# chongchen1999/llm-inference-engine

Measured on AMD Instinct MI355X. Metric: decode_tokens_per_s, higher is better.
Workload: dtype f16; 1 GPU; Llama-2-7B 32-layer fp16 decode, batch 1, ctx 2048 (BASELINE configs[2]); random-init weights, synthetic ids, KV pre-filled; global_batch=1, seq_len=2048, parallelism=replicas x1 (no collective), graph=True, layers=32

## Files before the change

### include/llmie.h

```cpp
#ifndef LLMIE_H
#define LLMIE_H

#include <stddef.h>
#include <stdint.h>

#ifdef __cplusplus
extern "C" {
#endif

#define LLMIE_ABI_VERSION 3

typedef enum { LLMIE_F32 = 0, LLMIE_F16 = 1 } llmie_dtype;

typedef enum {
    LLMIE_OK = 0,
    LLMIE_ERR_INVALID_ARG = -1,
    LLMIE_ERR_UNSUPPORTED = -2,
    LLMIE_ERR_LAUNCH = -3,
    LLMIE_ERR_WORKSPACE = -4
} llmie_status;

typedef void *llmie_stream;

typedef enum {
// ... 159 lines not shown
    int32_t *out_top_ids;
    float   *out_top_logprobs;
} llmie_sampling_ext;
int llmie_sample_logits_ext(const void *logits, int batch, int vocab, const llmie_sampling_params *params_dev, int32_t *history,
                            int history_stride, int32_t *history_len, int history_append, int32_t *seq_len, uint8_t *finished,
                            int32_t *out_id, float *out_logprob, int step, const int32_t *step_dev, int end_id, void *workspace,
                            size_t workspace_bytes, llmie_dtype dtype, llmie_stream stream, const llmie_sampling_ext *ext);

size_t llmie_score_tokens_workspace_bytes(int rows, int hidden_size, int vocab);
int llmie_score_tokens(const void *hidden, const void *norm_gamma, float rms_eps, const void *lm_head, const void *lm_bias,
                       const int32_t *targets, float *out_logprob, float *out_lse, int32_t *out_argmax,
                       float *out_argmax_logprob, int rows, int hidden_size, int vocab, void *workspace,
                       size_t workspace_bytes, llmie_dtype dtype, llmie_stream stream);


int llmie_linear_w8a16(const void *x, const int8_t *wq, const void *scale, void *y,
                       int M, int K, int N, const void *bias, const void *residual,
                       void *workspace, size_t workspace_bytes, llmie_stream stream);
int llmie_linear_w4a16(const void *x, const uint8_t *wq, const void *scale, void *y,
                       int M, int K, int N, int group, const void *bias, const void *residual,
                       void *workspace, size_t workspace_bytes, llmie_stream stream);
int llmie_linear_fp8(const void *x, const uint8_t *w_fp8, const float *w_scale, void *y,
                     int M, int K, int N, const void *bias, const void *residual,
                     void *workspace, size_t workspace_bytes, llmie_stream stream);
size_t llmie_linear_fp8_workspace_bytes(int M, int K, int N);
int llmie_linear_fp8_swiglu(const void *x, const uint8_t *w_fp8, const float *w_scale, void *y, int M, int K,
                            int two_inter, void *workspace, size_t workspace_bytes, llmie_stream stream);
int llmie_quantize_w8(const void *w, int8_t *wq, void *scale, int N, int K, llmie_stream stream);
int llmie_quantize_w4(const void *w, uint8_t *wq, void *scale, int N, int K, int group,
                      llmie_stream stream);
int llmie_quantize_fp8(const void *w, uint8_t *wq, float *scale, int N, int K, llmie_stream stream);

int llmie_quantize_mxfp4(const void *w, uint8_t *wq, uint8_t *scale, int N, int K, llmie_stream stream);
int llmie_dequantize_mxfp4(const uint8_t *wq, const uint8_t *scale, void *w16, int N, int K, llmie_stream stream);
int llmie_linear_mxfp4(const void *x, const uint8_t *wq, const uint8_t *scale, void *y, int M, int K, int N, const void *bias,
                       const void *residual, void *workspace, size_t workspace_bytes, llmie_stream stream);

size_t llmie_packed_weight_bytes(llmie_weight_format fmt, int N, int K, int swiglu_pairs);
size_t llmie_packed_scale_bytes(llmie_weight_format fmt, int N, int K, int swiglu_pairs);
int llmie_pack_weight(llmie_weight_format fmt, const void *w, const void *scale, void *packed, void *packed_scale,
                      int N, int K, int swiglu_pairs, llmie_stream stream);
size_t llmie_linear_packed_workspace_bytes(llmie_weight_format fmt, int M, int K, int N);
enum { LLMIE_X32_X = 1, LLMIE_X32_Y = 2, LLMIE_X32_RES = 4 };
size_t llmie_x32_bytes(int C);
int llmie_x32_convert(const void *src, void *dst, int M, int C, int to_x32, llmie_stream stream);
int llmie_linear_packed(llmie_weight_format fmt, const void *x, const void *packed, const void *scale, void *y,
                        int M, int K, int N, int swiglu, int x32_flags, const void *residual, const void *gamma,
                        const void *pre_bias, float eps, void *workspace, size_t workspace_bytes,
                        llmie_stream stream);


typedef enum { LLMIE_KV_NATIVE = 0, LLMIE_KV_FP8 = 1 } llmie_kv_format;

typedef struct {
    const void *data;
    const void *scale;
    const void *bias;
} llmie_matrix;

typedef struct {
    const void *attn_norm_gamma;
    llmie_matrix qkv;
    llmie_matrix o;
    const void *ffn_norm_gamma;
    llmie_matrix gate_up;
    llmie_matrix down;
} llmie_layer_weights;

typedef struct {
    int head_num, kv_head_num, head_size, inter_size, num_layers, vocab_size;
    int max_seq_len, max_batch;
    int rotary_dim;
    float rotary_base, rms_eps;
    llmie_dtype dtype;
    llmie_weight_format wfmt;
    int int4_group;
    llmie_kv_format kv_fmt;
    float k_scale, v_scale;
    int flags;
} llmie_decoder_config;

#define LLMIE_DEC_NO_PACKED_COPY 1
#define LLMIE_DEC_PACKED_ONLY 2
size_t llmie_decoder_resident_weight_bytes(const llmie_decoder_config *cfg);

#define LLMIE_PLAN_PAGED 1u
#define LLMIE_PLAN_RAGGED 2u
#define LLMIE_PLAN_HIDDEN_MISALIGNED 4u
#define LLMIE_PLAN_WEIGHTS_MISALIGNED 8u
#define LLMIE_PLAN_GAMMAS_MISALIGNED 16u
#define LLMIE_PLAN_O_BIAS 32u
#define LLMIE_PLAN_SCALES_MISALIGNED 64u
#define LLMIE_SW_NO_FUSED_DECODE 1u
#define LLMIE_SW_NO_FUSED_BATCH 2u
#define LLMIE_SW_NO_PACKED_BATCH 4u
#define LLMIE_SW_CHAIN 8u
#define LLMIE_SW_NO_FUSED_SHORT_PREFILL 16u
#define LLMIE_SW_NO_QKV_ROPE_FUSION 32u
const char *llmie_decoder_plan_name(const llmie_decoder_config *cfg, int prefill, int rows, unsigned call_flags, unsigned switch_mask);

#define LLMIE_PLAN_QKV_BIAS_MISALIGNED 128u
#define LLMIE_PLAN_GATE_UP_SCALES_MISALIGNED 256u
#define LLMIE_PLAN_NO_FFN_GAMMA 512u
const char *llmie_decoder_prefill_layer_plan(const llmie_decoder_config *cfg, int tokens, int batch, int max_q_len, unsigned call_flags,
                                             unsigned switch_mask, int *status);

typedef struct llmie_decoder llmie_decoder;

size_t llmie_decoder_workspace_bytes(const llmie_decoder_config *cfg);
llmie_decoder *llmie_decoder_create(const llmie_decoder_config *cfg,
                                    const llmie_layer_weights *layers,
                                    void *workspace, size_t workspace_bytes);
void llmie_decoder_destroy(llmie_decoder *dec);
int llmie_decoder_repack(llmie_decoder *dec, const llmie_layer_weights *layers, llmie_stream stream);

int llmie_decoder_forward(llmie_decoder *dec, const void *hidden_in, void *hidden_out,
                          void *k_cache, void *v_cache, int batch, int step,
                          const int32_t *step_dev, llmie_stream stream);

#define LLMIE_KV_PAGE_TOKENS 128
int llmie_decoder_forward_paged(llmie_decoder *dec, const void *hidden_in, void *hidden_out, void *k_pool, void *v_pool,
                                const int32_t *block_table, int max_pages, int num_pages, int batch, int step,
                                const int32_t *step_dev, llmie_stream stream);
int llmie_decoder_forward_ragged(llmie_decoder *dec, const void *hidden_in, void *hidden_out, void *k_cache, void *v_cache,
                                 int batch, const int32_t *ctx_len_dev, llmie_stream stream);
int llmie_decoder_forward_paged_ragged(llmie_decoder *dec, const void *hidden_in, void *hidden_out, void *k_pool, void *v_pool,
                                       const int32_t *block_table, int max_pages, int num_pages, int batch,
                                       const int32_t *ctx_len_dev, llmie_stream stream);
int llmie_decoder_prefill_paged(llmie_decoder *dec, const void *hidden_in, void *hidden_out, void *k_pool, void *v_pool,
                                const int32_t *block_table, int max_pages, int num_pages, const int32_t *input_lengths,
                                const int32_t *history_lengths, int batch, int num_tokens, int max_q_len, void *workspace,
                                size_t workspace_bytes, llmie_stream stream);
int llmie_kv_pages_copy(void *dense, void *pool, const int32_t *block_table, const int32_t *ctx_len, int to_pages,
                        int layers, int batch, int kv_head_num, int max_seq_len, int head_size, int max_pages,
                        int num_pages, int elem_bytes, llmie_stream stream);

#define LLMIE_BEAM_MAX_WIDTH 16
size_t llmie_beam_step_workspace_bytes(int groups, int width, int vocab);
int llmie_beam_step(const void *logits , int groups, int width, int vocab,
                    float *cum_logprob , int32_t *gen_len ,
                    uint8_t *finished , int32_t *out_parent ,
                    int32_t *out_token , int end_id, float length_penalty, void *workspace,
                    size_t workspace_bytes, llmie_dtype dtype, llmie_stream stream);

size_t llmie_kv_pages_fork_workspace_bytes(int rows, int layers, int kv_head_num, int head_size, int elem_bytes, int max_pages);
int llmie_kv_pages_fork(void *k_pool, void *v_pool, int32_t *block_table ,
                        const int32_t *own_table , const int32_t *parent ,
                        int32_t *cached_len , int rows, int layers, int kv_head_num, int head_size,
                        int max_pages, int num_pages, int elem_bytes, void *workspace, size_t workspace_bytes,
                        llmie_stream stream);

#define LLMIE_SPEC_MAX_DRAFT 15
size_t llmie_spec_verify_workspace_bytes(int batch, int k, int vocab);
int llmie_spec_verify(const void *logits , int batch, int k, int vocab,
                      const int32_t *draft_ids , const int32_t *draft_len ,
                      const llmie_sampling_params *params_dev , int32_t *history, int history_stride,
                      int32_t *history_len, int history_append, int32_t *seq_len, uint8_t *finished,
                      int32_t *out_tokens , int32_t *out_count , float *out_logprob ,
                      int32_t *last_token , int32_t *cached_len ,
                      int32_t *step_rows , int step, const int32_t *step_dev, int end_id,
                      void *workspace, size_t workspace_bytes, llmie_dtype dtype, llmie_stream stream,
                      const llmie_sampling_ext *ext );

int llmie_ngram_draft(const int32_t *tokens , int stride, const int32_t *len ,
                      const uint8_t *finished , int batch, int k, int max_n, int min_n, int pad_id,
                      int32_t *out_ids , int32_t *out_draft_ids ,
                      int32_t *out_draft_len , llmie_stream stream);

#define LLMIE_LORA_MAX_SLOTS 1024
#define LLMIE_LORA_MAX_KSPLIT 8
#define LLMIE_LORA_QKV 0
#define LLMIE_LORA_O 1
#define LLMIE_LORA_GATE_UP 2
#define LLMIE_LORA_DOWN 3
typedef struct {
    const void *a[4];
    const void *b[4];
} llmie_lora_layer;
typedef struct {
    int rank;
    float scale;
    int layers;
    const llmie_lora_layer *layer;
} llmie_lora_adapter;
size_t llmie_lora_table_bytes(int slots, int layers);
int llmie_lora_slot_load(void *table_dev, int slots, int layers, int slot, const llmie_lora_adapter *host_desc, llmie_stream stream);
size_t llmie_lora_workspace_bytes(int max_rows, int slots, int max_rank_total);
int llmie_lora_plan(const int32_t *slot_dev, const int32_t *lengths_dev , int batch, int rows, const void *table_dev,
                    int slots, void *workspace, size_t workspace_bytes, llmie_stream stream);
int llmie_lora_apply(const void *x , void *y , int rows, int K, int N, int blocks,
                     const int *block_widths , const void *table_dev, int slots, int layers, int layer, int module,
                     void *workspace, size_t workspace_bytes, llmie_dtype dtype, llmie_stream stream);

#define LLMIE_PLAN_LORA 1024u
size_t llmie_decoder_lora_workspace_bytes(const llmie_decoder_config *cfg, int max_tokens, int slots);
int llmie_decoder_lora_attach(llmie_decoder *dec, const void *table_dev, int slots, const int32_t *seq_slot_dev, void *workspace,
                              size_t workspace_bytes);
int llmie_decoder_lora_detach(llmie_decoder *dec);

size_t llmie_decoder_prefill_workspace_bytes(const llmie_decoder_config *cfg, int max_tokens, int max_batch);
int llmie_decoder_prefill(llmie_decoder *dec, const void *hidden_in, void *hidden_out, void *k_cache, void *v_cache,
                          const int32_t *input_lengths, const int32_t *history_lengths, int batch, int num_tokens,
                          int max_q_len, void *workspace, size_t workspace_bytes, llmie_stream stream);

int llmie_lm_head_sample(llmie_decoder *dec, void *hidden ,
                         const void *final_norm_gamma, const llmie_matrix *lm_head,
                         llmie_weight_format lm_fmt, void *logits,
                         int32_t *tmp_ids, void *tmp_vals, int32_t *topk_ids, void *topk_vals,
                         int K, int blocks_per_row, int32_t *seq_len, uint8_t *finished,
                         int32_t *out_ids, int batch, int step, const int32_t *step_dev,
                         int end_id, llmie_stream stream);

int llmie_lm_head_sample_next(llmie_decoder *dec, void *hidden, const void *final_norm_gamma, const llmie_matrix *lm_head,
                              llmie_weight_format lm_fmt, void *logits, int32_t *tmp_ids, void *tmp_vals, int32_t *topk_ids,
                              void *topk_vals, int K, int blocks_per_row, int32_t *seq_len, uint8_t *finished, int32_t *out_ids,
                              int batch, int step, int32_t *step_dev, int end_id, const void *embed_table, void *next_hidden,
                              int advance_step, llmie_stream stream);

int llmie_lm_head_sample_params(llmie_decoder *dec, void *hidden, const void *final_norm_gamma, const llmie_matrix *lm_head,
                                llmie_weight_format lm_fmt, void *logits, const llmie_sampling_params *params_dev, int32_t *history,
                                int history_stride, int32_t *history_len, int history_append, int32_t *seq_len, uint8_t *finished,
                                int32_t *out_ids, float *out_logprob, int batch, int step, int32_t *step_dev, int end_id,
                                const void *embed_table, void *next_hidden, int advance_step, void *workspace, size_t workspace_bytes,
                                llmie_stream stream);

int llmie_lm_head_sample_ext(llmie_decoder *dec, void *hidden, const void *final_norm_gamma, const llmie_matrix *lm_head,
                             llmie_weight_format lm_fmt, void *logits, const llmie_sampling_params *params_dev, int32_t *history,
                             int history_stride, int32_t *history_len, int history_append, int32_t *seq_len, uint8_t *finished,
                             int32_t *out_ids, float *out_logprob, int batch, int step, int32_t *step_dev, int end_id,
                             const void *embed_table, void *next_hidden, int advance_step, void *workspace, size_t workspace_bytes,
                             llmie_stream stream, const llmie_sampling_ext *ext);

enum {
    LLMIE_OP_ATTN_NORM = 0, LLMIE_OP_QKV_GEMM, LLMIE_OP_ROPE, LLMIE_OP_MHA, LLMIE_OP_O_GEMM,
    LLMIE_OP_FFN_NORM, LLMIE_OP_GATE_UP_SWIGLU, LLMIE_OP_DOWN_GEMM, LLMIE_OP_FINAL_NORM,
    LLMIE_OP_LM_HEAD, LLMIE_OP_TOPK, LLMIE_OP_SAMPLING,
    LLMIE_OP_CHAIN,
    LLMIE_OP_COUNT
};
int llmie_decoder_profile_begin(llmie_decoder *dec, int max_events);
int llmie_decoder_profile_end(llmie_decoder *dec, llmie_stream stream, double *ms_by_op ,
                              int *launches_by_op );

int llmie_decoder_status(llmie_decoder *dec, llmie_stream stream);
int llmie_decoder_debug_stamps(llmie_decoder *dec, void *stamps_dev);

int llmie_advance_step(int32_t *step_dev, llmie_stream stream);

#ifdef __cplusplus
}
#endif
#endif
```

### llm-inference-engine_amd/__init__.py

```python
import ctypes as C
import os

_HERE = os.path.dirname(os.path.abspath(__file__))
LIB_PATH = os.path.join(_HERE, "lib", "libllmie.so")

F32, F16 = 0, 1
W_F16, W_INT8, W_INT4, W_FP8, W_F32 = 0, 1, 2, 3, 4
W_MXFP4 = 5
KV_NATIVE, KV_FP8 = 0, 1
DEC_NO_PACKED_COPY, DEC_PACKED_ONLY = 1, 2
ABI_VERSION = 3

_lib = None


class LlmieError(RuntimeError):
    pass


def build(force=False, jobs=4):
    import importlib.util
    spec = importlib.util.spec_from_file_location("llmie_amd_build", os.path.join(_HERE, "build.py"))
    mod = importlib.util.module_from_spec(spec)
    spec.loader.exec_module(mod)
    return mod.build(force=force, jobs=jobs)


_vp, _i, _f, _sz = C.c_void_p, C.c_int, C.c_float, C.c_size_t

_SIGS = {
    "llmie_input_embedding": [_vp, _vp, _vp, _i, _i, _i, _i, _vp],
    "llmie_cal_padding_offset": [_vp, _vp, _vp, _i, _i, _vp],
    "llmie_build_causal_mask": [_vp, _vp, _vp, _i, _i, _i, _i, _vp],
    "llmie_rmsnorm": [_vp, _vp, _vp, _f, _i, _i, _i, _vp],
    "llmie_fused_add_bias_residual_rmsnorm": [_vp, _vp, _vp, _vp, _f, _i, _i, _i, _vp],
    "llmie_add_residual": [_vp, _vp, _i, _i, _i, _vp],
    "llmie_linear_workspace_bytes": [_i, _i, _i, _i],
    "llmie_linear": [_vp, _vp, _vp, _i, _i, _i, _i, _vp, _vp, _i, _vp, _sz, _vp],
    "llmie_linear_swiglu": [_vp, _vp, _vp, _i, _i, _i, _i, _vp, _sz, _vp],
    "llmie_linear_route": [_i, _vp, _vp, _vp, _vp, _i, _i, _i, _i, _i, _vp, _vp, _vp, _sz],
    "llmie_gemm256_tiles": [_i, _i, _i, _i, _i],
    "llmie_batched_gemm": [_vp, _vp, _vp, _i, _i, _i, _i, _i, _i, _vp],
    "llmie_qkv_bias_transpose_rope": [_vp, _vp, _vp, _vp, _vp, _vp, _vp, _i, _i, _i, _i, _i, _i, _i, _f, _i, _vp],
    "llmie_rope_decode": [_vp, _i, _i, _i, _i, _i, _vp, _i, _f, _i, _vp],
    "llmie_decoder_mha_workspace_bytes": [_i, _i, _i, _i],
    "llmie_decoder_mha": [_vp, _vp, _vp, _vp, _vp, _i, _i, _i, _i, _i, _i, _i, _vp, _vp, _sz, _i, _vp],
    "llmie_decoder_mha_rope": [_vp, _vp, _vp, _vp, _vp, _i, _i, _i, _i, _i, _i, _i, _vp, _vp, _sz, _vp, _i, _vp, _i,
                               _vp],
    "llmie_concat_kv": [_vp, _vp, _vp, _vp, _i, _i, _i, _i, _i, _i, _i, _vp],
    "llmie_repeat_kv": [_vp, _vp, _vp, _i, _i, _i, _i, _i, _i, _i, _i, _vp],
    "llmie_scale_mask_softmax": [_vp, _vp, _vp, _f, _i, _i, _i, _i, _i, _vp],
    "llmie_transpose_remove_padding": [_vp, _vp, _vp, _i, _i, _i, _i, _i, _i, _vp],
    "llmie_silu_and_mul": [_vp, _vp, _i, _i, _i, _vp],
    "llmie_topk": [_vp, _vp, _vp, _vp, _vp, _i, _i, _i, _i, _i, _vp],
    "llmie_sampling": [_vp, _vp, _vp, _vp, _vp, _i, _i, _i, _vp, _i, _i, _i, _vp],
    "llmie_linear_w8a16": [_vp, _vp, _vp, _vp, _i, _i, _i, _vp, _vp, _vp, _sz, _vp],
    "llmie_linear_w4a16": [_vp, _vp, _vp, _vp, _i, _i, _i, _i, _vp, _vp, _vp, _sz, _vp],
    "llmie_linear_fp8": [_vp, _vp, _vp, _vp, _i, _i, _i, _vp, _vp, _vp, _sz, _vp],
    "llmie_linear_fp8_workspace_bytes": [_i, _i, _i],
    "llmie_linear_fp8_swiglu": [_vp, _vp, _vp, _vp, _i, _i, _i, _vp, _sz, _vp],
    "llmie_packed_weight_bytes": [_i, _i, _i, _i],
    "llmie_packed_scale_bytes": [_i, _i, _i, _i],
    "llmie_pack_weight": [_i, _vp, _vp, _vp, _vp, _i, _i, _i, _vp],
    "llmie_linear_packed_workspace_bytes": [_i, _i, _i, _i],
    "llmie_linear_packed": [_i, _vp, _vp, _vp, _vp, _i, _i, _i, _i, _i, _vp, _vp, _vp, _f, _vp, _sz, _vp],
    "llmie_x32_bytes": [_i],
    "llmie_x32_convert": [_vp, _vp, _i, _i, _i, _vp],
    "llmie_quantize_w8": [_vp, _vp, _vp, _i, _i, _vp],
    "llmie_quantize_w4": [_vp, _vp, _vp, _i, _i, _i, _vp],
    "llmie_quantize_fp8": [_vp, _vp, _vp, _i, _i, _vp],
    "llmie_quantize_mxfp4": [_vp, _vp, _vp, _i, _i, _vp],
    "llmie_dequantize_mxfp4": [_vp, _vp, _vp, _i, _i, _vp],
    "llmie_linear_mxfp4": [_vp, _vp, _vp, _vp, _i, _i, _i, _vp, _vp, _vp, _sz, _vp],
    "llmie_decoder_workspace_bytes": [_vp],
    "llmie_decoder_create": [_vp, _vp, _vp, _sz],
    "llmie_decoder_destroy": [_vp],
    "llmie_decoder_forward": [_vp, _vp, _vp, _vp, _vp, _i, _i, _vp, _vp],
    "llmie_decoder_forward_ragged": [_vp, _vp, _vp, _vp, _vp, _i, _vp, _vp],
    "llmie_decoder_forward_paged_ragged": [_vp, _vp, _vp, _vp, _vp, _vp, _i, _i, _i, _vp, _vp],
    "llmie_decoder_mha_plan": [_i, _i, _i, _i, _i, _i, _i, _i, C.c_uint, _i, _i, C.c_ulonglong, C.c_longlong, _vp],
    "llmie_decoder_mha_ragged": [_vp, _vp, _vp, _vp, _vp, _i, _i, _i, _i, _i, _i, _vp, _vp, _sz, _vp, _i, _vp, _i, _i, _i, _vp],
    "llmie_decoder_prefill_workspace_bytes": [_vp, _i, _i],
    "llmie_decoder_prefill": [_vp, _vp, _vp, _vp, _vp, _vp, _vp, _i, _i, _i, _vp, _sz, _vp],
    "llmie_lm_head_sample": [_vp, _vp, _vp, _vp, _i, _vp, _vp, _vp, _vp, _vp, _i, _i, _vp, _vp, _vp, _i, _i, _vp,
                             _i, _vp],
    "llmie_lm_head_sample_next": [_vp, _vp, _vp, _vp, _i, _vp, _vp, _vp, _vp, _vp, _i, _i, _vp, _vp, _vp, _i, _i, _vp, _i, _vp, _vp,
                                  _i, _vp],
    "llmie_advance_step": [_vp, _vp],
    "llmie_sample_logits_workspace_bytes": [_i, _i],
    "llmie_sample_logits": [_vp, _i, _i, _vp, _vp, _i, _vp, _i, _vp, _vp, _vp, _vp, _i, _vp, _i, _vp, _sz, _i, _vp],
    "llmie_sample_logits_ext": [_vp, _i, _i, _vp, _vp, _i, _vp, _i, _vp, _vp, _vp, _vp, _i, _vp, _i, _vp, _sz, _i, _vp, _vp],
    "llmie_score_tokens_workspace_bytes": [_i, _i, _i],
    "llmie_score_tokens": [_vp, _vp, _f, _vp, _vp, _vp, _vp, _vp, _vp, _vp, _i, _i, _i, _vp, _sz, _i, _vp],
    "llmie_lm_head_sample_params": [_vp, _vp, _vp, _vp, _i, _vp, _vp, _vp, _i, _vp, _i, _vp, _vp, _vp, _vp, _i, _i, _vp, _i, _vp,
                                    _vp, _i, _vp, _sz, _vp],
    "llmie_lm_head_sample_ext": [_vp, _vp, _vp, _vp, _i, _vp, _vp, _vp, _i, _vp, _i, _vp, _vp, _vp, _vp, _i, _i, _vp, _i, _vp,
                                 _vp, _i, _vp, _sz, _vp, _vp],
    "llmie_decoder_forward_paged": [_vp, _vp, _vp, _vp, _vp, _vp, _i, _i, _i, _i, _vp, _vp],
    "llmie_decoder_prefill_paged": [_vp, _vp, _vp, _vp, _vp, _vp, _i, _i, _vp, _vp, _i, _i, _i, _vp, _sz, _vp],
    "llmie_kv_pages_copy": [_vp, _vp, _vp, _vp, _i, _i, _i, _i, _i, _i, _i, _i, _i, _vp],
    "llmie_beam_step_workspace_bytes": [_i, _i, _i],
    "llmie_beam_step": [_vp, _i, _i, _i, _vp, _vp, _vp, _vp, _vp, _i, _f, _vp, _sz, _i, _vp],
    "llmie_kv_pages_fork_workspace_bytes": [_i, _i, _i, _i, _i, _i],
    "llmie_kv_pages_fork": [_vp, _vp, _vp, _vp, _vp, _vp, _i, _i, _i, _i, _i, _i, _i, _vp, _sz, _vp],
    "llmie_spec_verify_workspace_bytes": [_i, _i, _i],
    "llmie_spec_verify": [_vp, _i, _i, _i, _vp, _vp, _vp, _vp, _i, _vp, _i, _vp, _vp, _vp, _vp, _vp, _vp, _vp, _vp, _i, _vp, _i, _vp, _sz,
                          _i, _vp, _vp],
    "llmie_ngram_draft": [_vp, _i, _vp, _vp, _i, _i, _i, _i, _i, _vp, _vp, _vp, _vp],
    "llmie_lora_table_bytes": [_i, _i],
    "llmie_lora_slot_load": [_vp, _i, _i, _i, _vp, _vp],
    "llmie_lora_workspace_bytes": [_i, _i, _i],
    "llmie_lora_plan": [_vp, _vp, _i, _i, _vp, _i, _vp, _sz, _vp],
    "llmie_lora_apply": [_vp, _vp, _i, _i, _i, _i, _vp, _vp, _i, _i, _i, _i, _vp, _sz, _i, _vp],
    "llmie_decoder_lora_workspace_bytes": [_vp, _i, _i],
    "llmie_decoder_lora_attach": [_vp, _vp, _i, _vp, _vp, _sz],
    "llmie_decoder_lora_detach": [_vp],
    "llmie_decoder_profile_begin": [_vp, _i],
    "llmie_decoder_profile_end": [_vp, _vp, _vp, _vp],
    "llmie_decoder_status": [_vp, _vp],
    "llmie_decoder_resident_weight_bytes": [_vp],
    "llmie_decoder_repack": [_vp, _vp, _vp],
    "llmie_decoder_plan_name": [_vp, _i, _i, C.c_uint, C.c_uint],
    "llmie_decoder_prefill_layer_plan": [_vp, _i, _i, _i, C.c_uint, C.c_uint, _vp],
    "llmie_decoder_debug_stamps": [_vp, _vp],
    "llmie_abi_version": [],
    "llmie_last_error": [],
    "llmie_target_arch": [],
}
_RESTYPES = {
    "llmie_decoder_mha_workspace_bytes": _sz,
    "llmie_decoder_resident_weight_bytes": _sz,
    "llmie_linear_fp8_workspace_bytes": _sz,
    "llmie_linear_workspace_bytes": _sz,
    "llmie_packed_weight_bytes": _sz,
    "llmie_x32_bytes": _sz,
    "llmie_packed_scale_bytes": _sz,
    "llmie_linear_packed_workspace_bytes": _sz,
    "llmie_decoder_workspace_bytes": _sz,
    "llmie_decoder_prefill_workspace_bytes": _sz,
    "llmie_sample_logits_workspace_bytes": _sz,
    "llmie_score_tokens_workspace_bytes": _sz,
    "llmie_beam_step_workspace_bytes": _sz,
    "llmie_kv_pages_fork_workspace_bytes": _sz,
    "llmie_spec_verify_workspace_bytes": _sz,
    "llmie_lora_table_bytes": _sz,
    "llmie_lora_workspace_bytes": _sz,
    "llmie_decoder_lora_workspace_bytes": _sz,
    "llmie_decoder_create": _vp,
    "llmie_decoder_destroy": None,
    "llmie_last_error": C.c_char_p,
    "llmie_linear_route": C.c_char_p,
    "llmie_gemm256_tiles": C.c_char_p,
    "llmie_decoder_mha_plan": C.c_char_p,
    "llmie_decoder_plan_name": C.c_char_p,
    "llmie_decoder_prefill_layer_plan": C.c_char_p,
    "llmie_target_arch": C.c_char_p,
}

EXPORTS = tuple(sorted(_SIGS))


def lib():
    global _lib
    if _lib is None:
        if not os.path.exists(LIB_PATH):
            raise LlmieError(
                "HIP library %s is missing: run `python llm-inference-engine_amd/build.py` "
                "(or __graft_entry__.build()).  There is no CPU fallback." % LIB_PATH)
        import torch
        l = C.CDLL(LIB_PATH)
        for name, args in _SIGS.items():
            fn = getattr(l, name)
            fn.argtypes = args
            fn.restype = _RESTYPES.get(name, C.c_int)
        if l.llmie_abi_version() != ABI_VERSION:
            raise LlmieError("libllmie.so ABI version %d, this binding was written against %d (include/llmie.h)"
                             % (l.llmie_abi_version(), ABI_VERSION))
        _lib = l
    return _lib


def _check(rc, what):
    if rc != 0:
        raise LlmieError("%s failed (%d): %s" % (what, rc, lib().llmie_last_error().decode()))


def _dt(t):
    import torch
    if t.dtype == torch.float32:
        return F32
    if t.dtype == torch.float16:
        return F16
    raise LlmieError("unsupported dtype %s" % t.dtype)


def _p(t):
    if t is None:
        return None
    assert t.is_cuda and t.is_contiguous(), "device-resident contiguous tensors only"
    return t.data_ptr()


def _st():
    import torch
    return torch.cuda.current_stream().cuda_stream


def input_embedding(ids, table, out):
    _check(lib().llmie_input_embedding(_p(ids), _p(table), _p(out), ids.numel(), table.shape[1], table.shape[0],
                                       _dt(table), _st()), "input_embedding")
    return out

# ... 492 lines not shown
        need = lib().llmie_decoder_prefill_workspace_bytes(C.byref(self.cfg), T, bs)
        if getattr(self, "_pf_ws", None) is None or self._pf_ws.numel() < need:
            self._pf_ws = torch.empty(need, dtype=torch.uint8, device="cuda")
        _check(lib().llmie_decoder_prefill_paged(self.handle, _p(hidden_in), _p(hidden_out), _p(k_pool), _p(v_pool),
                                                 _p(block_table), block_table.shape[1], k_pool.shape[1], _p(input_lengths),
                                                 _p(history_lengths), bs, T, max_q_len, self._pf_ws.data_ptr(),
                                                 self._pf_ws.numel(), _st()), "decoder_prefill_paged")
        return hidden_out

    def lm_head_sample(self, hidden, final_gamma, lm_head, lm_fmt, logits, tmp_ids, tmp_vals, topk_ids, topk_vals,
                       seq_len, finished, out_ids, step, end_id, blocks_per_row=8, step_dev=None, embed=None, next_hidden=None,
                       advance=False, fused_tail=False):
        m = _mat(lm_head)
        if fused_tail or embed is not None or advance:
            _check(lib().llmie_lm_head_sample_next(self.handle, _p(hidden), _p(final_gamma), C.byref(m), lm_fmt, _p(logits),
                                                   _p(tmp_ids), _p(tmp_vals), _p(topk_ids), _p(topk_vals), topk_ids.shape[-1],
                                                   blocks_per_row, _p(seq_len), _p(finished), _p(out_ids), hidden.shape[0], step,
                                                   _p(step_dev), end_id, _p(embed), _p(next_hidden), 1 if advance else 0, _st()),
                   "lm_head_sample_next")
            return
        _check(lib().llmie_lm_head_sample(self.handle, _p(hidden), _p(final_gamma), C.byref(m), lm_fmt, _p(logits),
                                          _p(tmp_ids), _p(tmp_vals), _p(topk_ids), _p(topk_vals),
                                          topk_ids.shape[-1], blocks_per_row, _p(seq_len), _p(finished), _p(out_ids),
                                          hidden.shape[0], step, _p(step_dev), end_id, _st()), "lm_head_sample")

    def lm_head_sample_params(self, hidden, final_gamma, lm_head, lm_fmt, logits, params, seq_len, finished, out_ids, step,
                              end_id, history=None, history_len=None, append=False, out_logprob=None, step_dev=None, embed=None,
                              next_hidden=None, advance=False, workspace=None, ext=None):
        m = _mat(lm_head)
        bs = hidden.shape[0]
        ws, ws_bytes = _sample_ws(workspace, bs, self.cfg.vocab_size, hidden.device)
        stride = 0 if history is None else history.shape[1]
        args = (self.handle, _p(hidden), _p(final_gamma), C.byref(m), lm_fmt, _p(logits), _p(params), _p(history), stride,
                _p(history_len), 1 if append else 0, _p(seq_len), _p(finished), _p(out_ids), _p(out_logprob), bs, step,
                _p(step_dev), end_id, _p(embed), _p(next_hidden), 1 if advance else 0, _p(ws), ws_bytes, _st())
        if ext is None:
            _check(lib().llmie_lm_head_sample_params(*args), "lm_head_sample_params")
        else:
            _check(lib().llmie_lm_head_sample_ext(*args, _ext_ref(ext)), "lm_head_sample_ext")

    OPS = ("attn_norm", "qkv_gemm", "rope", "mha", "o_gemm", "ffn_norm", "gate_up_swiglu", "down_gemm",
           "final_norm", "lm_head", "topk", "sampling", "chain")

    def lora_workspace_bytes(self, max_tokens, slots):
        return lib().llmie_decoder_lora_workspace_bytes(C.byref(self.cfg), max_tokens, slots)

    def lora_attach(self, table, seq_slot, max_tokens=None, workspace=None):
        import torch
        assert table.layers == self.cfg.num_layers, "the table must have the engine's layer count"
        need = self.lora_workspace_bytes(max_tokens or self.cfg.max_batch, table.slots)
        if workspace is None:
            workspace = torch.empty(max(need, 256), dtype=torch.uint8, device=table.data.device)
        _check(lib().llmie_decoder_lora_attach(self.handle, _p(table.data), table.slots, _p(seq_slot), _p(workspace), workspace.numel()),
               "decoder_lora_attach")
        self._lora_keep = (table, seq_slot, workspace)
        return workspace

    def lora_detach(self):
        _check(lib().llmie_decoder_lora_detach(self.handle), "decoder_lora_detach")
        self._lora_keep = None

    def profile_begin(self, max_events):
        _check(lib().llmie_decoder_profile_begin(self.handle, max_events), "decoder_profile_begin")

    def profile_end(self):
        ms = (C.c_double * len(self.OPS))()
        n = (C.c_int * len(self.OPS))()
        _check(lib().llmie_decoder_profile_end(self.handle, _st(), ms, n), "decoder_profile_end")
        return {op: (ms[i], n[i]) for i, op in enumerate(self.OPS)}

    def repack(self, layers):
        arr = (LayerWeights * len(layers))()
        for i, lw in enumerate(layers):
            arr[i] = LayerWeights(_p(lw["attn_norm"]), _mat(lw["qkv"]), _mat(lw["o"]), _p(lw["ffn_norm"]), _mat(lw["gate_up"]), _mat(lw["down"]))
        _check(lib().llmie_decoder_repack(self.handle, arr, _st()), "decoder_repack")
        self._keep = layers

    def debug_stamps(self, buf):
        _check(lib().llmie_decoder_debug_stamps(self.handle, _p(buf)), "decoder_debug_stamps")

    def status(self):
        _check(lib().llmie_decoder_status(self.handle, _st()), "decoder_status")

    def close(self):
        if self.handle:
            lib().llmie_decoder_destroy(self.handle)
            self.handle = None

    def __del__(self):
        try:
            self.close()
        except Exception:
            pass


LORA_MODULES = ("qkv", "o", "gate_up", "down")
LORA_RANKS = (8, 16, 32, 64)
LORA_MAX_SLOTS = 1024
LORA_MAX_KSPLIT = 8
PLAN_LORA = 1024
PLAN_PAGED, PLAN_RAGGED, PLAN_HIDDEN_MISALIGNED = 1, 2, 4


class LoraLayer(C.Structure):
    _fields_ = [("a", _vp * 4), ("b", _vp * 4)]


class LoraAdapter(C.Structure):
    _fields_ = [("rank", _i), ("scale", _f), ("layers", _i), ("layer", C.POINTER(LoraLayer))]


class LoraTable:

    def __init__(self, data, slots, layers):
        self.data, self.slots, self.layers = data, slots, layers
        self.keep = [None] * slots


def lora_table(slots, layers, device="cuda"):
    import torch
    n = lib().llmie_lora_table_bytes(slots, layers)
    if n == 0:
        raise LlmieError("lora_table: bad shape slots=%d layers=%d" % (slots, layers))
    return LoraTable(torch.zeros(n, dtype=torch.uint8, device=device), slots, layers)


def _lora_stack(m, parts):
    import torch
    if m is None:
        m = parts
    if m is None or (isinstance(m, (tuple, list)) and all(x is None for x in m)):
        return None
    if any(x is None for x in m):
        raise LlmieError("lora_slot_load: a fused module needs the adapter of every block (pass zero matrices for a missing one), "
                         "and every A its B")
    if isinstance(m[0], (tuple, list)):
        return torch.cat([x[0] for x in m], 0).contiguous(), torch.cat([x[1] for x in m], 0).contiguous()
    return m[0].contiguous(), m[1].contiguous()


def lora_slot_load(table, slot, adapter, scale=1.0):
    if adapter is None:
        _check(lib().llmie_lora_slot_load(_p(table.data), table.slots, table.layers, slot, None, _st()), "lora_slot_load")
        if 0 <= slot < table.slots:
            table.keep[slot] = (table.keep[slot][1] or table.keep[slot][0] if table.keep[slot] else None, None)
        return
    arr = (LoraLayer * len(adapter))()
    keep, rank = [], 0
    for i, lw in enumerate(adapter):
        sep = {"qkv": ("q", "k", "v"), "gate_up": ("gate", "up")}
        for mo, name in enumerate(LORA_MODULES):
            parts = [lw.get(k) for k in sep[name]] if name in sep else None
            ab = _lora_stack(lw.get(name), parts)
            if ab is None:
                continue
            keep.append(ab)
            rank = rank or ab[1].shape[1]
            if ab[1].shape[1] != rank or ab[0].shape[0] % rank:
                raise LlmieError("lora_slot_load: layer %d module %s has rank %d (A rows %d), the adapter's first module has %d"
                                 % (i, name, ab[1].shape[1], ab[0].shape[0], rank))
            arr[i].a[mo], arr[i].b[mo] = _p(ab[0]), _p(ab[1])
    desc = LoraAdapter(rank, scale, len(adapter), arr)
    _check(lib().llmie_lora_slot_load(_p(table.data), table.slots, table.layers, slot, C.byref(desc), _st()), "lora_slot_load")
    table.keep[slot] = (table.keep[slot][1] or table.keep[slot][0] if table.keep[slot] else None, keep)


# ... 244 lines not shown
```

### llm-inference-engine_amd/csrc/attention_decode.hip

```cpp
#include "llmie_internal.h"

#include <cstdlib>
#include <type_traits>

namespace llmie {

struct fp8kv_t {
    uint8_t b;
};
template <typename KT> struct CacheVec {
    using type = typename Vec16<KT>::type;
    static constexpr int n = Vec16<KT>::n;
};
template <> struct CacheVec<fp8kv_t> {
    using type = uint4_t;
    static constexpr int n = 16;
};
template <typename KT, int N> __device__ __forceinline__ void kv_to_f32(const typename CacheVec<KT>::type &v, float (&o)[N]) {
    if constexpr (std::is_same<KT, fp8kv_t>::value) {
#pragma unroll
        for (int w = 0; w < 4; ++w) {
            const auto lo = __builtin_amdgcn_cvt_pk_f32_fp8(static_cast<int>(v[w]), false);
            const auto hi = __builtin_amdgcn_cvt_pk_f32_fp8(static_cast<int>(v[w]), true);
            o[4 * w] = lo[0];
            o[4 * w + 1] = lo[1];
            o[4 * w + 2] = hi[0];
            o[4 * w + 3] = hi[1];
        }
    } else {
#pragma unroll
        for (int e = 0; e < N; ++e) o[e] = to_f32(v[e]);
    }
}
template <typename KT, typename T, int N> __device__ __forceinline__ typename CacheVec<KT>::type kv_pack(const T (&x)[N], float inv_scale) {
    typename CacheVec<KT>::type v;
    if constexpr (std::is_same<KT, fp8kv_t>::value) {
#pragma unroll
        for (int w = 0; w < 4; ++w)
            v[w] = pack4_e4m3(to_f32(x[4 * w]) * inv_scale, to_f32(x[4 * w + 1]) * inv_scale, to_f32(x[4 * w + 2]) * inv_scale,
                              to_f32(x[4 * w + 3]) * inv_scale);
    } else {
#pragma unroll
        for (int e = 0; e < N; ++e) v[e] = x[e];
    }
    return v;
}
template <typename T, int N> __device__ __forceinline__ void load_elems(const T *p, T (&dst)[N]) {
    constexpr int PER = Vec16<T>::n;
    static_assert(N % PER == 0, "whole 16-byte loads");
#pragma unroll
    for (int c = 0; c < N / PER; ++c) {
        const typename Vec16<T>::type v = reinterpret_cast<const typename Vec16<T>::type *>(p)[c];
#pragma unroll
        for (int e = 0; e < PER; ++e) dst[c * PER + e] = v[e];
    }
}

template <typename KT, int HS, int NWV = 4, int GL = 8> struct AttnGeom {
    static constexpr int N = CacheVec<KT>::n;
    static constexpr int LPT = HS / N;
    static constexpr int TPW = 64 / LPT;
    static constexpr int CHUNK = NWV * GL * TPW;
};

__host__ __device__ inline int attn_min_chunk() { return 32; }

struct QkvSlabs {
    const float *slab;
    int KS;
    size_t stride;
    SlabScale sc;
};

constexpr int KV_PAGE = 128;
struct PagedKv {
    const int32_t *table;
    int max_pages;
    int step_stride;
    int out_x32;
};
__device__ __forceinline__ int seq_step(const int32_t *step_dev, int step_arg, int stride, int b, int max_seq_len) {
    const int s = step_dev ? step_dev[static_cast<size_t>(b) * stride] : step_arg;
    return (s >= 1 && s <= max_seq_len) ? s : 0;
}
__device__ __forceinline__ size_t attn_out_index(int x32, int b, int k, int width) {
    if (!x32) return static_cast<size_t>(b) * width + k;
    return (static_cast<size_t>(k >> 5) * 2 + (b >> 4)) * 512 + ((k & 31) >> 3) * 128 + (b & 15) * 8 + (k & 7);
}

__device__ __forceinline__ void merge_round(const float (&ms)[16], const float (&ls)[16], const float (&os)[16], int s0, int nsplits,
                                            float &M, float &L, float &o) {
    float Mc = M;
#pragma unroll
    for (int i = 0; i < 16; ++i)
        if (s0 + i < nsplits) Mc = fmaxf(Mc, ms[i]);
    const float rescale = (M == -INFINITY) ? 0.f : __expf(M - Mc);
    L *= rescale;
    o *= rescale;
#pragma unroll
    for (int i = 0; i < 16; ++i)
        if (s0 + i < nsplits) {
            const float f = __expf(ms[i] - Mc);
            L = fmaf(f, ls[i], L);
            o = fmaf(f, os[i], o);
        }
    M = Mc;
}
__device__ __forceinline__ void merge_load(const float *__restrict__ p, int s0, int last, size_t stride, int d, float (&ms)[16],
                                           float (&ls)[16], float (&os)[16]) {
#pragma unroll
    for (int i = 0; i < 16; ++i) {
        const int s = min(s0 + i, last);
        ms[i] = p[s * stride];
        ls[i] = p[s * stride + 1];
        os[i] = p[s * stride + 2 + d];
    }
}
__device__ __forceinline__ float merge_splits(const float *__restrict__ p, int nsplits, size_t stride, int d) {
    float M = -INFINITY, L = 0.f, o = 0.f;
    for (int s0 = 0; s0 < nsplits; s0 += 16) {
        float ms[16], ls[16], os[16];
        merge_load(p, s0, nsplits - 1, stride, d, ms, ls, os);
        merge_round(ms, ls, os, s0, nsplits, M, L, o);
    }
    return o / (L + 1e-6f);
}

template <typename T, int HS, int REP, int kAttnWaves = 4, int kAttnG = 8, typename KT = T>
__global__ __launch_bounds__(kAttnWaves * 64) void decode_attn_split_kernel(
    const T *__restrict__ qkv, const T *__restrict__ qkv_bias, KT *k_cache, KT *v_cache,
    float *__restrict__ part, T *__restrict__ out, int head_num, int kv_head_num, int max_seq_len,
    int step_arg, const int32_t *__restrict__ step_dev, int max_splits,
    const float2 *__restrict__ rope , int rotary_dim,
    int32_t *tickets ,
    const QkvSlabs qs ,
    const float k_scale, const float v_scale ,
    const PagedKv pg ,
    const int cpw ) {
    using G = AttnGeom<KT, HS, kAttnWaves, kAttnG>;
    using V = typename CacheVec<KT>::type;
    constexpr int N = G::N, LPT = G::LPT, TPW = G::TPW, CHUNK = G::CHUNK;
    constexpr int NT = kAttnWaves * 64;
    constexpr bool FP8KV = std::is_same<KT, fp8kv_t>::value;
    static_assert(HS % N == 0 && LPT >= 1 && LPT <= 64 && (LPT & (LPT - 1)) == 0, "head size");

    const int split = blockIdx.x, g = blockIdx.y, b = blockIdx.z;
    const int step = seq_step(step_dev, step_arg, pg.step_stride, b, max_seq_len);
    const int span = cpw * CHUNK;
    const int t0 = split * span;
    if (t0 >= step) return;
    int tc0 = t0;
    int t_end = min(step, tc0 + CHUNK);
    const int nsplits = (step + span - 1) / span;
    const int batch = gridDim.z;

    const int lane = threadIdx.x & 63, wave = threadIdx.x >> 6;
    const int sub = lane / LPT, dl = lane % LPT;
    const int qkv_heads = head_num + 2 * kv_head_num;
    const float scale = rsqrtf(static_cast<float>(HS));

    const T *row = qkv + static_cast<size_t>(b) * qkv_heads * HS;
    constexpr int NPG = CHUNK > KV_PAGE ? CHUNK / KV_PAGE : 1;
    static_assert(CHUNK % KV_PAGE == 0 || KV_PAGE % CHUNK == 0, "chunk vs page size");
    int pg0 = 0;
    KT *kbase[NPG], *vbase[NPG];
    auto set_pages = [&]() {
        pg0 = tc0 / KV_PAGE;
#pragma unroll
        for (int j = 0; j < NPG; ++j) {
            size_t off;
            if (pg.table) {
                const int page = pg.table[static_cast<size_t>(b) * pg.max_pages + min(pg0 + j, pg.max_pages - 1)];
                off = (static_cast<size_t>(page) * kv_head_num + g) * KV_PAGE * HS;
            } else {
                off = (static_cast<size_t>(b) * kv_head_num + g) * max_seq_len * HS + static_cast<size_t>(pg0 + j) * KV_PAGE * HS;
            }
            kbase[j] = k_cache + off;
            vbase[j] = v_cache + off;
        }
    };
    set_pages();
    auto krow = [&](int t) { return kbase[NPG == 1 ? 0 : (t / KV_PAGE - pg0)] + static_cast<size_t>(t % KV_PAGE) * HS; };
    auto vrow = [&](int t) { return vbase[NPG == 1 ? 0 : (t / KV_PAGE - pg0)] + static_cast<size_t>(t % KV_PAGE) * HS; };
    KT *kc = kbase[0];
    const int t_new = step - 1;
    T qraw[REP][N];
    constexpr int ITEMS_PER_HEAD = HS / 4;
    constexpr int LROUNDS = ((REP + 2) * ITEMS_PER_HEAD + NT - 1) / NT;
    __shared__ __attribute__((aligned(16))) T qkvlds[(REP + 2) * HS];
    const bool wg_has_new = t_new >= t0 && t_new < t0 + span;
    floatx4 spart[LROUNDS][4];
    half4_t sscale[LROUNDS];
    floatx4 sscalef[LROUNDS];
    const float xs_b = (qs.slab && qs.sc.wf) ? qs.sc.xs[b] : 1.f;
    size_t scol[LROUNDS];
    bool sact[LROUNDS];
    if (qs.slab) {
#pragma unroll
        for (int lr = 0; lr < LROUNDS; ++lr) {
            const int item = lr * NT + threadIdx.x;
            const int hsel = item / ITEMS_PER_HEAD, d4 = item - hsel * ITEMS_PER_HEAD;
            sact[lr] = hsel < REP || (wg_has_new && hsel < REP + 2);
            const int hh = hsel < REP ? g * REP + hsel : (hsel == REP ? head_num + g : head_num + kv_head_num + g);
            scol[lr] = static_cast<size_t>(hh) * HS + d4 * 4;
            if (sact[lr]) {
                const float *p = qs.slab + static_cast<size_t>(b) * qkv_heads * HS + scol[lr];
#pragma unroll
                for (int kk = 0; kk < 4; ++kk)
// ... 437 lines not shown
    if (c.kv_e4m3)
        while (p.cpw < 8 && c.batch * c.kv_head_num >= 128 * p.cpw) p.cpw *= 2;
    const int base = c.kv_e4m3 ? attn_chunk<fp8kv_t>(p.hs) : (c.dtype == LLMIE_F32 ? attn_chunk<float>(p.hs) : attn_chunk<half_t>(p.hs));
    p.chunk = p.cpw * base;
    p.grid[0] = (bound + p.chunk - 1) / p.chunk, p.grid[1] = c.kv_head_num, p.grid[2] = c.batch;
    p.max_splits_ws = (c.max_seq_len + attn_min_chunk() - 1) / attn_min_chunk();
    p.merge = p.grid[0] > 1 && !c.tickets;
    p.merge_grid[0] = c.head_num, p.merge_grid[1] = c.batch;
    p.merge_block = p.hs < 64 ? 64 : p.hs;
    p.workspace_bytes = need;
    return p;
}

DecodeAttnPlan plan_decode_attn(const DecodeAttnCall &c) {
    if (c.ragged && !c.step_dev) return attn_refusal(DAREF_RAGGED_LENGTHS);
    if (c.out_x32 && (c.batch > 32 || c.dtype != LLMIE_F16)) return attn_refusal(DAREF_X32);
    if (c.paged && (c.max_pages <= 0 || c.num_pages <= 0 || static_cast<long long>(c.max_pages) * KV_PAGE < c.max_seq_len))
        return attn_refusal(DAREF_PAGES);
    if (c.slabs && (c.mis_wh8 || c.mis_wf || c.mis_slab || c.slab_stride_mod4)) return attn_refusal(DAREF_SLAB_ALIGNMENT);
    const int rep = c.head_num / c.kv_head_num;
    const bool aligned = !(c.mis_qkv | c.mis_k | c.mis_v | c.mis_bias);
    const size_t need = llmie_decoder_mha_workspace_bytes(c.batch, c.head_num, c.head_size, c.max_seq_len);
    const bool ws_ok = c.workspace && c.workspace_bytes >= need;
    if (c.kv_e4m3) {
        if (c.dtype != LLMIE_F16 || c.tickets) return attn_refusal(DAREF_E4M3_FORM);
        if (!aligned || !ws_ok || c.batch > 65535 || !c.scales_positive || (rep != 1 && rep != 2 && rep != 4) ||
            (c.head_size != 128 && c.head_size != 64))
            return attn_refusal(DAREF_E4M3, need);
        return plan_attn_split(c, need);
    }
    const bool geometry = attn_fused_geometry(c);
    if (aligned && c.batch <= 65535 && c.kv_head_num <= 65535 && geometry)
        return ws_ok ? plan_attn_split(c, need) : attn_refusal(DAREF_WORKSPACE, need);
    if (c.paged) return attn_refusal(DAREF_PAGED_GEOMETRY);
    if (c.slabs) return attn_refusal(DAREF_SLABS_GEOMETRY);
    if (c.rope || (c.tickets && !geometry)) return attn_refusal(DAREF_ROPE_GEOMETRY);
    if (c.ragged || c.out_x32) return attn_refusal(DAREF_RAGGED_GEOMETRY);
    DecodeAttnPlan p{};
    p.lds_bytes = sizeof(float) * static_cast<size_t>(c.step_dev ? c.max_seq_len : c.step);
    if (p.lds_bytes > 60 * 1024) return attn_refusal(DAREF_GENERIC_SPAN);
    p.kind = DA_GENERIC, p.grid[0] = c.head_num, p.grid[1] = c.batch, p.grid[2] = 1;
    return p;
}

int decode_attn_refuse(const DecodeAttnCall &c, const DecodeAttnPlan &p) {
    const char *fused = "head_size in {32,64,128,256} and head_num/kv_head_num in {1,2,4,8}";
    switch (p.refusal) {
        case DAREF_RAGGED_LENGTHS: set_error("decoder_mha: a ragged batch needs the device array of context lengths"); return LLMIE_ERR_INVALID_ARG;
        case DAREF_X32: set_error("decoder_mha: the x32 output image holds at most 32 fp16 rows"); break;
        case DAREF_PAGES: set_error("decoder_mha: paged KV cache needs max_pages * %d >= max_seq_len and num_pages > 0", KV_PAGE); break;
        case DAREF_SLAB_ALIGNMENT: set_error("decoder_mha: q/k/v from split-K slabs needs 16-byte aligned slabs and aligned scale vectors"); break;
        case DAREF_E4M3_FORM: set_error("decoder_mha(fp8 KV): fp16 activations, separate merge kernel only"); break;
        case DAREF_E4M3:
            set_error("decoder_mha(fp8 KV): needs head_size 64/128, head ratio 1/2/4, 16-byte aligned buffers, positive scales and "
                      "the llmie_decoder_mha workspace");
            break;
        case DAREF_WORKSPACE:
            set_error("decoder_mha: workspace too small (%zu < %zu bytes)", c.workspace_bytes, p.workspace_bytes);
            return LLMIE_ERR_WORKSPACE;
        case DAREF_PAGED_GEOMETRY: set_error("decoder_mha: the paged KV cache needs %s", fused); break;
        case DAREF_SLABS_GEOMETRY: set_error("decoder_mha: q/k/v from split-K slabs needs %s", fused); break;
        case DAREF_ROPE_GEOMETRY: set_error("decoder_mha: fused RoPE / in-launch merge need %s", fused); break;
        case DAREF_RAGGED_GEOMETRY: set_error("decoder_mha: ragged batches / x32 output need %s", fused); break;
        case DAREF_GENERIC_SPAN:
            set_error("decoder_mha: generic path supports at most 15360 tokens (head_size=%d, rep=%d)", c.head_size, c.head_num / c.kv_head_num);
            break;
        default: set_error("decoder_mha: refused"); break;
    }
    return LLMIE_ERR_UNSUPPORTED;
}

struct DecodeAttnArgs {
    const void *qkv, *bias;
    void *kc, *vc, *out;
    float *part;
    int head_num, kv_head_num, head_size, max_seq_len, step;
    const int32_t *step_dev;
    const float2 *rope;
    int rot_dim;
    int32_t *tickets;
    QkvSlabs qs;
    KvScale ks;
    PagedKv pg;
};

template <typename T, int HS, int REP, typename KT> static void launch_split(const DecodeAttnPlan &p, const DecodeAttnArgs &a, hipStream_t st) {
    decode_attn_split_kernel<T, HS, REP, 4, 8, KT><<<dim3(p.grid[0], p.grid[1], p.grid[2]), 4 * 64, 0, st>>>(
        static_cast<const T *>(a.qkv), static_cast<const T *>(a.bias), static_cast<KT *>(a.kc), static_cast<KT *>(a.vc), a.part,
        static_cast<T *>(a.out), a.head_num, a.kv_head_num, a.max_seq_len, a.step, a.step_dev, p.max_splits_ws, a.rope, a.rot_dim, a.tickets,
        a.qs, a.ks.k, a.ks.v, a.pg, p.cpw);
    if (p.merge)
        decode_attn_combine_kernel<T><<<dim3(p.merge_grid[0], p.merge_grid[1]), p.merge_block, 0, st>>>(
            a.part, static_cast<T *>(a.out), a.head_num, HS, p.chunk, a.step, a.step_dev, p.max_splits_ws, a.pg.step_stride, a.max_seq_len,
            a.pg.out_x32);
}
template <typename T> static void launch_generic(const DecodeAttnPlan &p, const DecodeAttnArgs &a, hipStream_t st) {
    decode_attn_generic_kernel<T><<<dim3(p.grid[0], p.grid[1]), 256, p.lds_bytes, st>>>(
        static_cast<const T *>(a.qkv), static_cast<const T *>(a.bias), static_cast<T *>(a.kc), static_cast<T *>(a.vc), static_cast<T *>(a.out),
        a.head_num, a.kv_head_num, a.head_size, a.max_seq_len, a.step, a.step_dev);
}
template <typename T, int HS, typename KT> static void launch_split_rep(const DecodeAttnPlan &p, const DecodeAttnArgs &a, hipStream_t st) {
    switch (p.rep) {
        case 1: return launch_split<T, HS, 1, KT>(p, a, st);
        case 2: return launch_split<T, HS, 2, KT>(p, a, st);
        case 4: return launch_split<T, HS, 4, KT>(p, a, st);
        case 8:
            if constexpr (std::is_same<KT, T>::value) return launch_split<T, HS, 8, KT>(p, a, st);
    }
}
template <typename T, typename KT> static void launch_split_hs(const DecodeAttnPlan &p, const DecodeAttnArgs &a, hipStream_t st) {
    switch (p.hs) {
        case 128: return launch_split_rep<T, 128, KT>(p, a, st);
        case 64: return launch_split_rep<T, 64, KT>(p, a, st);
        case 32:
            if constexpr (std::is_same<KT, T>::value) return launch_split_rep<T, 32, KT>(p, a, st);
            break;
        case 256:
            if constexpr (std::is_same<KT, T>::value) return launch_split_rep<T, 256, KT>(p, a, st);
            break;
    }
}
static int launch_decode_attn(const DecodeAttnCall &c, const DecodeAttnPlan &p, const DecodeAttnArgs &a, hipStream_t st) {
    const bool split = p.kind == DA_SPLIT;
    if (p.e4m3) launch_split_hs<half_t, fp8kv_t>(p, a, st);
    else if (c.dtype == LLMIE_F32) split ? launch_split_hs<float, float>(p, a, st) : launch_generic<float>(p, a, st);
    else split ? launch_split_hs<half_t, half_t>(p, a, st) : launch_generic<half_t>(p, a, st);
    return launch_status(p.e4m3 ? "decoder_mha(fp8 KV)" : "decoder_mha");
}

static size_t kv_layer_offset(const DecodeAttnShape &g, const KvView &kv, int layer) {
    return kv.block_table ? static_cast<size_t>(layer) * kv.num_pages * g.kv_head_num * KV_PAGE * g.head_size
                          : static_cast<size_t>(layer) * g.batch * g.kv_head_num * g.max_seq_len * g.head_size;
}
static DecodeAttnArgs decode_attn_args(const DecodeAttnShape &g, const DecodeAttnIo &io, const KvView &kv, const DecodePos &pos, int layer) {
    const size_t elem = kv.fp8 ? 1 : (g.dtype == LLMIE_F32 ? sizeof(float) : sizeof(half_t));
    const size_t layer_bytes = kv_layer_offset(g, kv, layer) * elem;
    QkvSlabs qs{nullptr, 0, 0, SlabScale{nullptr, nullptr, nullptr}};
    if (io.qkv_slabs)
        qs = QkvSlabs{io.qkv_slabs->slab, io.qkv_slabs->KS, static_cast<size_t>(io.qkv_slabs->M) * io.qkv_slabs->N,
                      io.qkv_scale ? *io.qkv_scale : SlabScale{nullptr, nullptr, nullptr}};
    return DecodeAttnArgs{io.qkv, io.qkv_bias, static_cast<char *>(kv.k) + layer_bytes, static_cast<char *>(kv.v) + layer_bytes, io.out,
                          static_cast<float *>(io.workspace), g.head_num, g.kv_head_num, g.head_size, g.max_seq_len, pos.step, pos.step_dev,
                          io.rope, io.rot_dim, io.tickets, qs, KvScale{kv.k_scale, kv.v_scale},
                          PagedKv{kv.block_table, kv.max_pages, pos.ragged ? 1 : 0, io.out_x32 ? 1 : 0}};
}
static DecodeAttnCall decode_attn_call(const DecodeAttnShape &g, const DecodeAttnIo &io, const KvView &kv, const DecodePos &pos,
                                       const DecodeAttnArgs &a) {
    DecodeAttnCall c{};
    c.dtype = g.dtype, c.kv_e4m3 = kv.fp8 != 0, c.scales_positive = kv.k_scale > 0.f && kv.v_scale > 0.f;
    c.head_size = g.head_size, c.head_num = g.head_num, c.kv_head_num = g.kv_head_num, c.batch = g.batch, c.max_seq_len = g.max_seq_len;
    c.step = pos.step, c.step_dev = pos.step_dev != nullptr, c.ragged = pos.ragged != 0;
    c.bias = io.qkv_bias != nullptr, c.rope = io.rope != nullptr, c.tickets = io.tickets != nullptr, c.slabs = io.qkv_slabs != nullptr;
    c.paged = kv.block_table != nullptr, c.out_x32 = io.out_x32 != 0, c.max_pages = kv.max_pages, c.num_pages = kv.num_pages;
    c.mis_qkv = mis16(a.qkv), c.mis_bias = mis16(a.bias), c.mis_k = mis16(a.kc), c.mis_v = mis16(a.vc);
    if (c.slabs) {
        c.mis_slab = mis16(a.qs.slab), c.mis_wf = mis16(a.qs.sc.wf), c.mis_wh8 = mis16(a.qs.sc.wh) % 8;
        c.slab_stride_mod4 = static_cast<unsigned>(a.qs.stride % 4);
    }
    c.workspace = io.workspace != nullptr, c.workspace_bytes = io.workspace_bytes;
    return c;
}

int decoder_mha_rope(const DecodeAttnShape &g, const DecodeAttnIo &io, const KvView &kv, const DecodePos &pos, int layer, hipStream_t st) {
    const DecodeAttnArgs a = decode_attn_args(g, io, kv, pos, layer);
    const DecodeAttnCall c = decode_attn_call(g, io, kv, pos, a);
    const DecodeAttnPlan p = plan_decode_attn(c);
    if (p.kind == DA_REFUSED) return decode_attn_refuse(c, p);
    return launch_decode_attn(c, p, a, st);
}

static int decode_attn_validate(const char *who, const DecodeAttnShape &g, const DecodePos &pos, bool pointers, int layer, bool rope, int rot_dim) {
    LLMIE_REQUIRE(pointers && (!pos.ragged || pos.step_dev), "%s: NULL pointer", who);
    LLMIE_REQUIRE(layer >= 0 && g.batch > 0 && g.head_num > 0 && g.kv_head_num > 0 && g.head_size > 0 && g.max_seq_len > 0, "%s: bad shape", who);
    LLMIE_REQUIRE(g.head_num % g.kv_head_num == 0, "%s: kv_head_num must divide head_num", who);
    LLMIE_REQUIRE(pos.step_dev || (pos.step >= 1 && pos.step <= g.max_seq_len), "%s: step %d outside [1, max_seq_len=%d]", who, pos.step,
                  g.max_seq_len);
    LLMIE_REQUIRE(!rope || (rot_dim > 0 && rot_dim % 2 == 0), "%s: bad rotary_dim", who);
    if (g.dtype != LLMIE_F32 && g.dtype != LLMIE_F16) LLMIE_UNSUPPORTED("%s: dtype %d", who, (int)g.dtype);
    return LLMIE_OK;
}
static int decode_attn_entry(const char *who, const DecodeAttnShape &g, const DecodeAttnIo &io, const KvView &kv, const DecodePos &pos, int layer,
                             llmie_stream stream) {
    const int rc = decode_attn_validate(who, g, pos, io.qkv && kv.k && kv.v && io.out, layer, io.rope != nullptr, io.rot_dim);
    return rc != LLMIE_OK ? rc : decoder_mha_rope(g, io, kv, pos, layer, as_stream(stream));
}

static void decode_attn_plan_text(const DecodeAttnCall &c, const DecodeAttnPlan &p, char *text, size_t n) {
    const char *dt = c.dtype == LLMIE_F32 ? "f32" : "f16";
    if (p.kind == DA_GENERIC) {
        snprintf(text, n, "generic %s grid %dx%d lds %zu", dt, p.grid[0], p.grid[1], p.lds_bytes);
        return;
    }
    const int k = snprintf(text, n, "split %s hs%d rep%d kv=%s cpw%d chunk%d grid %dx%dx%d merge ", dt, p.hs, p.rep, p.e4m3 ? "e4m3" : dt, p.cpw,
                           p.chunk, p.grid[0], p.grid[1], p.grid[2]);
    if (p.merge) snprintf(text + k, n - k, "%dx%d/%d", p.merge_grid[0], p.merge_grid[1], p.merge_block);
    else snprintf(text + k, n - k, "%s", p.grid[0] > 1 ? "in-launch" : "none");
}

}

using namespace llmie;

extern "C" size_t llmie_decoder_mha_workspace_bytes(int batch, int head_num, int head_size, int max_seq_len) {
    if (batch <= 0 || head_num <= 0 || head_size <= 0 || max_seq_len <= 0) return 0;
    const size_t splits = (static_cast<size_t>(max_seq_len) + attn_min_chunk() - 1) / attn_min_chunk();
    return static_cast<size_t>(batch) * head_num * splits * (head_size + 2) * sizeof(float);
}

extern "C" int llmie_decoder_mha(const void *qkv, const void *qkv_bias, void *k_cache, void *v_cache, void *out,
                                 int layer, int batch, int head_num, int kv_head_num, int head_size,
                                 int max_seq_len, int step, const int32_t *step_dev, void *workspace,
                                 size_t workspace_bytes, llmie_dtype dtype, llmie_stream stream) {
    return decode_attn_entry("decoder_mha", DecodeAttnShape{batch, head_num, kv_head_num, head_size, max_seq_len, dtype},
                             DecodeAttnIo{qkv, qkv_bias, out, workspace, workspace_bytes, nullptr, 0, nullptr, nullptr, nullptr, 0},
                             kv_dense(k_cache, v_cache), DecodePos{step, step_dev, 0}, layer, stream);
}

extern "C" int llmie_decoder_mha_rope(const void *qkv, const void *qkv_bias, void *k_cache, void *v_cache, void *out,
                                      int layer, int batch, int head_num, int kv_head_num, int head_size,
                                      int max_seq_len, int step, const int32_t *step_dev, void *workspace,
                                      size_t workspace_bytes, const void *rope_table, int rotary_dim, int32_t *tickets,
                                      llmie_dtype dtype, llmie_stream stream) {
    return decode_attn_entry("decoder_mha_rope", DecodeAttnShape{batch, head_num, kv_head_num, head_size, max_seq_len, dtype},
                             DecodeAttnIo{qkv, qkv_bias, out, workspace, workspace_bytes, static_cast<const float2 *>(rope_table), rotary_dim,
                                          tickets, nullptr, nullptr, 0},
                             kv_dense(k_cache, v_cache), DecodePos{step, step_dev, 0}, layer, stream);
}
// ... 41 lines not shown
```

### llm-inference-engine_amd/csrc/engine.hip

```cpp
#include "llmie_internal.h"

#include <cmath>
#include <cstdlib>
#include <new>
#include <vector>

using namespace llmie;

struct llmie_decoder {
    llmie_decoder_config cfg;
    std::vector<llmie_layer_weights> layers;
    int H, QKV, I;
    size_t esz;
    char *resid, *qkv, *mha, *act, *gu;
    void *attn_ws;
    size_t attn_ws_bytes;
    float2 *rope_table;
    void *fp8_ws;
    size_t fp8_ws_bytes;
    SlabWs slab_ws;
    unsigned *tail_ticket = nullptr;
    struct PackedLayer {
        const unsigned char *qkv, *o, *gate_up, *down;
        const void *sc[4];
    };
    std::vector<PackedLayer> packed;
    int pk_wf = 0;
    bool packed_only = false;
    half_t *hx = nullptr, *actx = nullptr;
    half_t *mhax = nullptr;
    float *pk_slab = nullptr;
    size_t pk_slab_floats = 0;
    unsigned char *pk_base = nullptr;
    unsigned *pk_sync = nullptr, *pk_err = nullptr;
    unsigned long long *pk_stamps = nullptr;
    struct Lora {
        const void *table = nullptr;
        int slots = 0;
        const int32_t *seq_slot = nullptr;
        void *ws = nullptr;
        size_t ws_bytes = 0;
    } lora;
    bool profiling = false;
    std::vector<hipEvent_t> ev;
    std::vector<int> ev_op;
    size_t ev_used = 0;
};

struct OpTimer {
    llmie_decoder *d;
    hipStream_t st;
    bool on;
    size_t idx;
    OpTimer(llmie_decoder *dec, int op, llmie_stream s) : d(dec), st(as_stream(s)), on(false), idx(0) {
        if (d->profiling && d->ev_used + 1 <= d->ev_op.size()) {
            idx = d->ev_used++;
            d->ev_op[idx] = op;
            on = hipEventRecord(d->ev[2 * idx], st) == hipSuccess;
        }
    }
    ~OpTimer() {
        if (on) (void)hipEventRecord(d->ev[2 * idx + 1], st);
    }
};
#define TIMED(op, expr)                 \
    do {                                \
        OpTimer _t(dec, op, stream);    \
        rc = (expr);                    \
    } while (0);                        \
    if (rc) return rc

static size_t align_up(size_t v) { return (v + 255) & ~static_cast<size_t>(255); }

static bool config_ok(const llmie_decoder_config *c) {
    if (!c) return false;
    if (c->head_num <= 0 || c->kv_head_num <= 0 || c->head_size <= 0 || c->inter_size <= 0 ||
        c->num_layers <= 0 || c->max_seq_len <= 0 || c->max_batch <= 0)
        return false;
    if (c->head_num % c->kv_head_num) return false;
    if (c->rotary_dim <= 0 || c->rotary_dim % 2) return false;
    if (c->dtype != LLMIE_F32 && c->dtype != LLMIE_F16) return false;
    if (c->dtype == LLMIE_F32 && c->wfmt != LLMIE_W_F32) return false;
    if (c->dtype == LLMIE_F16 && c->wfmt == LLMIE_W_F32) return false;
    if (c->wfmt == LLMIE_W_MXFP4 && ((c->head_num * c->head_size) % 32 || c->inter_size % 32)) return false;
    if (c->kv_fmt != LLMIE_KV_NATIVE && c->kv_fmt != LLMIE_KV_FP8) return false;
    if (c->flags & ~(LLMIE_DEC_NO_PACKED_COPY | LLMIE_DEC_PACKED_ONLY)) return false;
    if ((c->flags & LLMIE_DEC_NO_PACKED_COPY) && (c->flags & LLMIE_DEC_PACKED_ONLY)) return false;
    if (c->kv_fmt == LLMIE_KV_FP8) {
        const int rep = c->head_num / c->kv_head_num;
        if (c->dtype != LLMIE_F16 || (c->head_size != 128 && c->head_size != 64) || (rep != 1 && rep != 2 && rep != 4)) return false;
    }
    return true;
}

struct Carve {
    size_t off = 0;
    size_t take(size_t bytes) {
        const size_t o = off;
        off += align_up(bytes);
        return o;
    }
};

static int gemv_max_batch(llmie_weight_format wfmt) {
    switch (wfmt) {
        case LLMIE_W_F16: return 5;
        case LLMIE_W_INT8: return 2;
        case LLMIE_W_FP8: return 2;
        case LLMIE_W_INT4: return 2;
        default: return 4;
    }
}

static int packed_rows_max(const llmie_decoder_config &c) { return c.wfmt == LLMIE_W_FP8 ? 16 : 32; }
static bool packed_batch(const llmie_decoder_config &c, int batch) {
    return (batch > gemv_max_batch(c.wfmt) || (c.flags & LLMIE_DEC_PACKED_ONLY)) && batch <= packed_rows_max(c);
}

static int packed_wf(const llmie_decoder_config *c) {
    if (c->dtype != LLMIE_F16) return 0;
    const int wf = c->wfmt == LLMIE_W_F16 ? PKF_F16
                   : (c->wfmt == LLMIE_W_INT8 ? PKF_I8 : (c->wfmt == LLMIE_W_FP8 ? PKF_FP8 : (c->wfmt == LLMIE_W_INT4 && c->int4_group == 128 ? PKF_I4 : 0)));
    const bool only = (c->flags & LLMIE_DEC_PACKED_ONLY) != 0;
    if (!wf || (c->flags & LLMIE_DEC_NO_PACKED_COPY)) return 0;
    const int rows_max = packed_rows_max(*c);
    if (!packed_batch(*c, only || c->max_batch < rows_max ? c->max_batch : rows_max)) return 0;
    const int H = c->head_num * c->head_size, QKV = (c->head_num + 2 * c->kv_head_num) * c->head_size, I = c->inter_size;
    const int m = c->max_batch < 32 ? c->max_batch : 32;
    if (H % 32 || I % 32) return 0;
    if (!pk_eligible(wf, m, H, QKV, PKE_PLAIN) || !pk_eligible(wf, m, H, H, PKE_PLAIN) || !pk_eligible(wf, m, H, 2 * I, PKE_SWIGLU) ||
        !pk_eligible(wf, m, I, H, PKE_PLAIN))
        return 0;
    return wf;
}
static const char *packed_only_refusal(const llmie_decoder_config *c) {
    return c->wfmt == LLMIE_W_MXFP4 ? "decoder_create: LLMIE_DEC_PACKED_ONLY is not available for MXFP4 weights (no packed image is built)"
                                    : "decoder_create: LLMIE_DEC_PACKED_ONLY needs max_batch <= 32 (fp8: 16) and shapes / a format the packed kernels take";
}
struct PackedCarve {
    size_t per_layer[4], layer_bytes, hx, actx, mhax, slab, sync, total;
};
static PackedCarve packed_carve(const llmie_decoder_config *c, int wf) {
    PackedCarve p{};
    if (!wf) return p;
    const int H = c->head_num * c->head_size, QKV = (c->head_num + 2 * c->kv_head_num) * c->head_size, I = c->inter_size;
    p.per_layer[0] = align_up(pk_packed_bytes(wf, QKV, H, 0)) + align_up(pk_packed_scale_bytes(wf, QKV, H, 0));
    p.per_layer[1] = align_up(pk_packed_bytes(wf, H, H, 0)) + align_up(pk_packed_scale_bytes(wf, H, H, 0));
    p.per_layer[2] = align_up(pk_packed_bytes(wf, 2 * I, H, 1)) + align_up(pk_packed_scale_bytes(wf, 2 * I, H, 1));
    p.per_layer[3] = align_up(pk_packed_bytes(wf, H, I, 0)) + align_up(pk_packed_scale_bytes(wf, H, I, 0));
    p.layer_bytes = p.per_layer[0] + p.per_layer[1] + p.per_layer[2] + p.per_layer[3];
    p.hx = align_up(static_cast<size_t>(H) * 64);
    p.actx = align_up(static_cast<size_t>(I) * 64);
    p.mhax = p.hx;
    const int m = c->max_batch < 32 ? c->max_batch : 32;
    size_t sl = 0;
    for (int mm = 1; mm <= m; ++mm) {
        const size_t f = pk_slab_floats(wf, mm, I, H);
        sl = f > sl ? f : sl;
    }
    p.slab = align_up(sl * sizeof(float) + 16);
    p.sync = align_up(static_cast<size_t>(c->num_layers) * pk_chain_sync_bytes()) + 256;
    p.total = p.layer_bytes * c->num_layers + p.hx + p.actx + p.mhax + p.slab + p.sync;
    return p;
}
static size_t engine_slab_floats(const llmie_decoder_config *c, int rows) {
    int wbits;
    switch (c->wfmt) {
        case LLMIE_W_F16: wbits = 16; break;
        case LLMIE_W_INT8: wbits = 8; break;
// ... 86 lines not shown
    if (dec->pk_wf) rc = pack_layers(dec, layers, as_stream(stream));
    if (rc) return rc;
    dec->layers.assign(layers, layers + dec->cfg.num_layers);
    if (dec->packed_only)
        for (llmie_layer_weights &w : dec->layers) w.qkv.data = w.o.data = w.gate_up.data = w.down.data = nullptr;
    return LLMIE_OK;
}

extern "C" size_t llmie_decoder_resident_weight_bytes(const llmie_decoder_config *cfg) {
    if (!config_ok(cfg)) return 0;
    const size_t H = static_cast<size_t>(cfg->head_num) * cfg->head_size, QKV = static_cast<size_t>(cfg->head_num + 2 * cfg->kv_head_num) * cfg->head_size;
    const size_t I = cfg->inter_size, elems = QKV * H + H * H + 3 * H * I, rows = QKV + H + 2 * I + H;
    size_t row_major = 0, scales = 0;
    switch (cfg->wfmt) {
        case LLMIE_W_F16: row_major = elems * 2; break;
        case LLMIE_W_F32: row_major = elems * 4; break;
        case LLMIE_W_INT8: row_major = elems; scales = rows * 2; break;
        case LLMIE_W_FP8: row_major = elems; scales = rows * 4; break;
        case LLMIE_W_INT4: row_major = elems / 2; scales = (elems / (cfg->int4_group > 0 ? cfg->int4_group : 128)) * 2; break;
        case LLMIE_W_MXFP4: row_major = elems / 2; scales = elems / 32; break;
        default: return 0;
    }
    const int wf = packed_wf(cfg);
    const size_t images = wf ? packed_carve(cfg, wf).layer_bytes : 0;
    const size_t per_layer = ((cfg->flags & LLMIE_DEC_PACKED_ONLY) && wf ? 0 : row_major) + scales + images;
    return per_layer * cfg->num_layers;
}

extern "C" llmie_decoder *llmie_decoder_create(const llmie_decoder_config *cfg, const llmie_layer_weights *layers,
                                               void *workspace, size_t workspace_bytes) {
    if (!config_ok(cfg)) {
        set_error("decoder_create: invalid config");
        return nullptr;
    }
    if (!layers || !workspace) {
        set_error("decoder_create: NULL layers/workspace");
        return nullptr;
    }
    const EngineCarve offs = carve(cfg);
    const size_t need = offs.total;
    if (workspace_bytes < need) {
        set_error("decoder_create: workspace too small (%zu < %zu)", workspace_bytes, need);
        return nullptr;
    }
    if (reinterpret_cast<uintptr_t>(workspace) % 256) {
        set_error("decoder_create: workspace must be 256-byte aligned");
        return nullptr;
    }
    for (int l = 0; l < cfg->num_layers; ++l) {
        const llmie_layer_weights &w = layers[l];
        if (!w.attn_norm_gamma || !w.ffn_norm_gamma || !w.qkv.data || !w.o.data || !w.gate_up.data || !w.down.data) {
            set_error("decoder_create: layer %d has a NULL weight", l);
            return nullptr;
        }
        if (cfg->wfmt != LLMIE_W_F16 && cfg->wfmt != LLMIE_W_F32 &&
            (!w.qkv.scale || !w.o.scale || !w.gate_up.scale || !w.down.scale)) {
            set_error("decoder_create: layer %d lacks quantisation scales", l);
            return nullptr;
        }
    }
    llmie_decoder *d = new (std::nothrow) llmie_decoder();
    if (!d) return nullptr;
    d->cfg = *cfg;
    d->layers.assign(layers, layers + cfg->num_layers);
    d->H = cfg->head_num * cfg->head_size;
    d->QKV = (cfg->head_num + 2 * cfg->kv_head_num) * cfg->head_size;
    d->I = cfg->inter_size;
    d->esz = cfg->dtype == LLMIE_F16 ? 2 : 4;
    char *base = static_cast<char *>(workspace);
    d->resid = base + offs.resid;
    d->qkv = base + offs.qkv;
    d->mha = base + offs.mha;
    d->act = base + offs.act;
    d->gu = base + offs.gu;
    d->attn_ws = base + offs.attn_ws;
    d->attn_ws_bytes = llmie_decoder_mha_workspace_bytes(cfg->max_batch, cfg->head_num, cfg->head_size, cfg->max_seq_len);
    d->rope_table = reinterpret_cast<float2 *>(base + offs.rope_table);
    d->tail_ticket = reinterpret_cast<unsigned *>(base + offs.tail_ticket);
    if (hipMemset(d->tail_ticket, 0, 256) != hipSuccess) {
        set_error("decoder_create: clearing the workspace words failed");
        delete d;
        return nullptr;
    }
    d->fp8_ws = base + offs.fp8_ws;
    {
        const int kmax = cfg->inter_size > d->H ? cfg->inter_size : d->H;
        d->fp8_ws_bytes = cfg->wfmt == LLMIE_W_FP8 ? llmie_linear_fp8_workspace_bytes(cfg->max_batch, kmax, 0) : 0;
    }
    d->slab_ws = SlabWs{reinterpret_cast<float *>(base + offs.slabs), engine_slab_floats(cfg, cfg->max_batch)};
    if (!d->slab_ws.floats) d->slab_ws.p = nullptr;
    d->pk_wf = packed_wf(cfg);
    if ((cfg->flags & LLMIE_DEC_PACKED_ONLY) && !d->pk_wf) {
        set_error("%s", packed_only_refusal(cfg));
        delete d;
        return nullptr;
    }
    if (d->pk_wf) {
        if (hipDeviceSynchronize() != hipSuccess) {
            set_error("decoder_create: device synchronise failed");
            delete d;
            return nullptr;
        }
        const PackedCarve pc = packed_carve(cfg, d->pk_wf);
        unsigned char *pb = reinterpret_cast<unsigned char *>(base + offs.packed);
        d->pk_base = pb;
        const int prc = pack_layers(d, layers, nullptr);
        unsigned char *tail = pb + pc.layer_bytes * cfg->num_layers;
        d->hx = reinterpret_cast<half_t *>(tail);
        d->actx = reinterpret_cast<half_t *>(tail + pc.hx);
        d->mhax = reinterpret_cast<half_t *>(tail + pc.hx + pc.actx);
        d->pk_slab = reinterpret_cast<float *>(tail + pc.hx + pc.actx + pc.mhax);
        d->pk_slab_floats = (pc.slab - 16) / sizeof(float);
        d->pk_sync = reinterpret_cast<unsigned *>(tail + pc.hx + pc.actx + pc.mhax + pc.slab);
        d->pk_err = reinterpret_cast<unsigned *>(tail + pc.hx + pc.actx + pc.mhax + pc.slab + pc.sync - 256);
        if (prc != LLMIE_OK || hipMemset(tail, 0, pc.hx + pc.actx + pc.mhax) != hipSuccess || hipMemset(d->pk_sync, 0, pc.sync) != hipSuccess ||
            hipDeviceSynchronize() != hipSuccess) {
            set_error("decoder_create: packing the weights for the batch path failed");
            delete d;
            return nullptr;
        }
        if (cfg->flags & LLMIE_DEC_PACKED_ONLY) {
            d->packed_only = true;
            for (llmie_layer_weights &w : d->layers) w.qkv.data = w.o.data = w.gate_up.data = w.down.data = nullptr;
        }
    }
    {
        const int half = cfg->head_size / 2;
        std::vector<float2> tab(static_cast<size_t>(cfg->max_seq_len) * half);
        for (int pos = 0; pos < cfg->max_seq_len; ++pos)
            for (int j = 0; j < half; ++j) {
                float2 v{1.f, 0.f};
                if (j < cfg->rotary_dim / 2) {
                    const float ang = static_cast<float>(pos) / powf(cfg->rotary_base, static_cast<float>(2 * j) / static_cast<float>(cfg->rotary_dim));
                    v = float2{cosf(ang), sinf(ang)};
                }
                tab[static_cast<size_t>(pos) * half + j] = v;
            }
        if (hipMemcpy(d->rope_table, tab.data(), tab.size() * sizeof(float2), hipMemcpyHostToDevice) != hipSuccess) {
            set_error("decoder_create: RoPE table upload failed");
            delete d;
            return nullptr;
        }
    }
    return d;
}

extern "C" void llmie_decoder_destroy(llmie_decoder *dec) {
    if (!dec) return;
    for (hipEvent_t e : dec->ev) (void)hipEventDestroy(e);
    delete dec;
}

extern "C" int llmie_decoder_profile_begin(llmie_decoder *dec, int max_events) {
    LLMIE_REQUIRE(dec && max_events > 0, "decoder_profile_begin: bad arguments");
    while (dec->ev.size() < 2 * static_cast<size_t>(max_events)) {
        hipEvent_t e;
        if (hipEventCreate(&e) != hipSuccess) {
            set_error("decoder_profile_begin: hipEventCreate failed");
            return LLMIE_ERR_LAUNCH;
        }
        dec->ev.push_back(e);
    }
    dec->ev_op.assign(max_events, 0);
    dec->ev_used = 0;
    dec->profiling = true;
    return LLMIE_OK;
}

extern "C" int llmie_decoder_profile_end(llmie_decoder *dec, llmie_stream stream, double *ms_by_op, int *launches_by_op) {
    LLMIE_REQUIRE(dec && ms_by_op && launches_by_op, "decoder_profile_end: NULL pointer");
    dec->profiling = false;
    if (hipStreamSynchronize(as_stream(stream)) != hipSuccess) {
        set_error("decoder_profile_end: stream synchronise failed");
        return LLMIE_ERR_LAUNCH;
    }
    for (int i = 0; i < LLMIE_OP_COUNT; ++i) {
        ms_by_op[i] = 0.0;
        launches_by_op[i] = 0;
    }
    for (size_t i = 0; i < dec->ev_used; ++i) {
        float ms = 0.f;
        if (hipEventElapsedTime(&ms, dec->ev[2 * i], dec->ev[2 * i + 1]) == hipSuccess) {
            ms_by_op[dec->ev_op[i]] += ms;
            launches_by_op[dec->ev_op[i]] += 1;
        }
    }
    dec->ev_used = 0;
    return LLMIE_OK;
}

extern "C" int llmie_decoder_status(llmie_decoder *dec, llmie_stream stream) {
    LLMIE_REQUIRE(dec, "decoder_status: NULL decoder");
    if (hipStreamSynchronize(as_stream(stream)) != hipSuccess) {
        set_error("decoder_status: stream synchronise failed: %s", hipGetErrorString(hipGetLastError()));
        return LLMIE_ERR_LAUNCH;
    }
    if (!dec->pk_err) return LLMIE_OK;
    unsigned word = 0;
    if (hipMemcpy(&word, dec->pk_err, sizeof(word), hipMemcpyDeviceToHost) != hipSuccess) {
        set_error("decoder_status: reading the device error word failed");
        return LLMIE_ERR_LAUNCH;
    }
    if (word) {
        (void)hipMemset(dec->pk_err, 0, sizeof(word));
        (void)hipMemset(dec->pk_sync, 0, static_cast<size_t>(dec->cfg.num_layers) * pk_chain_sync_bytes());
        set_error("decoder: a grid barrier of the persistent chain launch timed out (code 0x%08x, phase %u): not every workgroup was "
                  "resident; set LLMIE_NO_CHAIN=1 to use the launch sequence", word, word & 0xfu);
        return LLMIE_ERR_LAUNCH;
    }
    return LLMIE_OK;
}

extern "C" int llmie_decoder_debug_stamps(llmie_decoder *dec, void *stamps_dev) {
    LLMIE_REQUIRE(dec, "decoder_debug_stamps: NULL decoder");
    dec->pk_stamps = static_cast<unsigned long long *>(stamps_dev);
    return LLMIE_OK;
}

static int engine_linear(const llmie_decoder *d, llmie_weight_format fmt, const void *x, const llmie_matrix &w,
                         void *y, int M, int K, int N, bool swiglu, const void *residual, bool use_bias,
                         llmie_stream stream) {
    const void *bias = use_bias ? w.bias : nullptr;
    switch (fmt) {
        case LLMIE_W_F16:
            return linear_f16_nk((const half_t *)x, (const half_t *)w.data, (half_t *)y, M, K, N,
                                 swiglu ? EPI_SWIGLU_ : EPI_NONE_, (const half_t *)bias, (const half_t *)residual, d->slab_ws,
                                 as_stream(stream));
        case LLMIE_W_F32:
            if (swiglu) {
                int rc = llmie_linear(x, w.data, d->gu, M, K, N, 1, bias, nullptr, LLMIE_F32, nullptr, 0, stream);
                if (rc) return rc;
                return llmie_silu_and_mul(d->gu, y, M, N / 2, LLMIE_F32, stream);
            }
            return llmie_linear(x, w.data, y, M, K, N, 1, bias, residual, LLMIE_F32, nullptr, 0, stream);
        case LLMIE_W_INT8:
        case LLMIE_W_INT4: {
            const int bits = fmt == LLMIE_W_INT8 ? 8 : 4;
            int rc = linear_wq(bits, (const half_t *)x, w.data, (const half_t *)w.scale, (half_t *)y, M, K, N, d->cfg.int4_group,
                               swiglu ? EPI_SWIGLU_ : EPI_NONE_, (const half_t *)bias, (const half_t *)residual, nullptr, nullptr,
                               0.f, d->slab_ws, as_stream(stream));
            return rc;
        }
        case LLMIE_W_FP8: {
            if (swiglu) {
                int rc = linear_fp8((const half_t *)x, (const uint8_t *)w.data, (const float *)w.scale, (half_t *)d->gu, M, K, N,
                                    (const half_t *)bias, nullptr, d->fp8_ws, d->fp8_ws_bytes, d->slab_ws, as_stream(stream));
                if (rc) return rc;
                return llmie_silu_and_mul(d->gu, y, M, N / 2, LLMIE_F16, stream);
            }
            return linear_fp8((const half_t *)x, (const uint8_t *)w.data, (const float *)w.scale, (half_t *)y, M, K, N,
                              (const half_t *)bias, (const half_t *)residual, d->fp8_ws, d->fp8_ws_bytes, d->slab_ws, as_stream(stream));
        }
        case LLMIE_W_MXFP4: {
            if (swiglu) {
                int rc = linear_mxfp4((const half_t *)x, (const uint8_t *)w.data, (const uint8_t *)w.scale, (half_t *)d->gu, M, K, N,
                                      (const half_t *)bias, nullptr, nullptr, 0, as_stream(stream));
                if (rc) return rc;
                return llmie_silu_and_mul(d->gu, y, M, N / 2, LLMIE_F16, stream);
            }
            return linear_mxfp4((const half_t *)x, (const uint8_t *)w.data, (const uint8_t *)w.scale, (half_t *)y, M, K, N,
                                (const half_t *)bias, (const half_t *)residual, nullptr, 0, as_stream(stream));
        }
        default:
            set_error("engine: weight format %d not supported by this build", (int)fmt);
            return LLMIE_ERR_UNSUPPORTED;
    }
}

struct EngineSwitches {
    bool no_fused_decode, no_fused_batch, no_packed_batch, chain, no_fused_short_prefill, no_qkv_rope_fusion;
};
static const EngineSwitches &engine_switches() {
    static const EngineSwitches s{getenv("LLMIE_NO_FUSED_DECODE") != nullptr,        getenv("LLMIE_NO_FUSED_BATCH") != nullptr,
                                  getenv("LLMIE_NO_PACKED_BATCH") != nullptr,        getenv("LLMIE_CHAIN") != nullptr,
                                  getenv("LLMIE_NO_FUSED_SHORT_PREFILL") != nullptr, getenv("LLMIE_NO_QKV_ROPE_FUSION") != nullptr};
    return s;
}
static EngineSwitches switches_of_mask(unsigned m) {
    return EngineSwitches{(m & LLMIE_SW_NO_FUSED_DECODE) != 0,        (m & LLMIE_SW_NO_FUSED_BATCH) != 0, (m & LLMIE_SW_NO_PACKED_BATCH) != 0,
                          (m & LLMIE_SW_CHAIN) != 0,                  (m & LLMIE_SW_NO_FUSED_SHORT_PREFILL) != 0,
                          (m & LLMIE_SW_NO_QKV_ROPE_FUSION) != 0};
}
static bool fused_attention_geometry(const llmie_decoder_config &c) {
    const int rep = c.head_num / c.kv_head_num;
    return (c.head_size == 32 || c.head_size == 64 || c.head_size == 128 || c.head_size == 256) && (rep == 1 || rep == 2 || rep == 4 || rep == 8);
}

enum DecodePath : int { DP_REFUSED = 0, DP_GEMV, DP_PACKED, DP_PACKED_CHAIN, DP_SPLITK, DP_UNFUSED, DP_LORA };
enum DecodeRefusal : int { DREF_NONE = 0, DREF_PACKED_ONLY, DREF_PAGED, DREF_KV_FP8, DREF_RAGGED, DREF_LORA, DREF_MX4_HIDDEN };
struct DecodeCall {
    llmie_decoder_config cfg;
    int batch;
    bool paged, ragged;
    unsigned mis_hidden, mis_wqkv0;
    EngineSwitches sw;
    bool lora;
};
static bool lora_engine_ok(const llmie_decoder_config &c) {
    const int H = c.head_num * c.head_size;
    return c.dtype == LLMIE_F16 && c.wfmt != LLMIE_W_FP8 && c.wfmt != LLMIE_W_F32 && c.wfmt != LLMIE_W_MXFP4 &&
           !(c.flags & LLMIE_DEC_PACKED_ONLY) && H % 32 == 0 &&
           c.inter_size % 32 == 0 && (c.kv_head_num * c.head_size) % 16 == 0;
}
static const char *const kLoraRefusal =
    "adapters need an fp16 engine with fp16 / int8 / int4 weights (an fp8-weight engine never materialises fp16 normalised rows, a "
    "LLMIE_DEC_PACKED_ONLY engine has no row-major route), hidden and inter sizes that are multiples of 32 and q / kv widths that are "
    "multiples of 16";
struct DecodePlan {
    int path, refusal;
    bool chain_wanted;
};
static DecodePlan plan_decode(const DecodeCall &d) {
    const llmie_decoder_config &c = d.cfg;
    const int batch = d.batch, H = c.head_num * c.head_size, I = c.inter_size;
    const bool attn_ok = fused_attention_geometry(c);
    const int wbits = c.wfmt == LLMIE_W_F16 ? 16 : (c.wfmt == LLMIE_W_INT8 ? 8 : (c.wfmt == LLMIE_W_INT4 ? 4 : 0));
    const bool fp8 = c.wfmt == LLMIE_W_FP8, packed_only = (c.flags & LLMIE_DEC_PACKED_ONLY) != 0;
    const int gemv_max = gemv_max_batch(c.wfmt);
    if (d.lora) {
        if (!lora_engine_ok(c)) return {DP_REFUSED, DREF_LORA, false};
        if (!attn_ok && d.paged) return {DP_REFUSED, DREF_PAGED, false};
        if (!attn_ok && c.kv_fmt == LLMIE_KV_FP8) return {DP_REFUSED, DREF_KV_FP8, false};
        if (!attn_ok && d.ragged) return {DP_REFUSED, DREF_RAGGED, false};
        return {DP_LORA, DREF_NONE, false};
    }
    if (c.wfmt == LLMIE_W_MXFP4) {
        if (packed_only) return {DP_REFUSED, DREF_PACKED_ONLY, false};
        if (d.mis_hidden) return {DP_REFUSED, DREF_MX4_HIDDEN, false};
        if (!attn_ok && d.paged) return {DP_REFUSED, DREF_PAGED, false};
        if (!attn_ok && c.kv_fmt == LLMIE_KV_FP8) return {DP_REFUSED, DREF_KV_FP8, false};
        if (!attn_ok && d.ragged) return {DP_REFUSED, DREF_RAGGED, false};
        return {DP_UNFUSED, DREF_NONE, false};
    }
    const bool int4_ok = wbits == 4 && c.int4_group == 128 && batch <= 64;
    const bool batch_path_ok = !d.sw.no_fused_batch && c.dtype == LLMIE_F16 && (wbits == 16 || wbits == 8 || int4_ok || fp8) && attn_ok &&
                               batch <= 128 && H % 256 == 0 && I % 256 == 0 && H >= 512 && I >= 512 && splitk_rownorm_eligible(H);
    const bool gemv_ok = !packed_only && (batch <= gemv_max || !batch_path_ok) &&
                         (wbits == 16 ? gemv_f16_eligible(batch, H, reinterpret_cast<const void *>(static_cast<uintptr_t>(d.mis_hidden)),
                                                          reinterpret_cast<const void *>(static_cast<uintptr_t>(d.mis_wqkv0)))
                                      : ((wbits != 0 || fp8) && ksplit_eligible(batch, H, fp8 ? 8 : wbits)));
    if (!d.sw.no_fused_decode && c.dtype == LLMIE_F16 && (wbits != 0 || fp8) && attn_ok && H % 8 == 0 && gemv_ok) return {DP_GEMV, DREF_NONE, false};
    const bool packed_on = !d.sw.no_packed_batch && !d.sw.no_fused_decode && attn_ok;
    if (packed_only && !(packed_on && packed_batch(c, batch))) return {DP_REFUSED, DREF_PACKED_ONLY, false};
    if (packed_on && packed_wf(&c) && packed_batch(c, batch)) return {DP_PACKED, DREF_NONE, d.sw.chain};
    if (batch_path_ok) return {DP_SPLITK, DREF_NONE, false};
    if (d.paged) return {DP_REFUSED, DREF_PAGED, false};
    if (c.kv_fmt == LLMIE_KV_FP8) return {DP_REFUSED, DREF_KV_FP8, false};
    if (d.ragged && !attn_ok) return {DP_REFUSED, DREF_RAGGED, false};
    return {DP_UNFUSED, DREF_NONE, false};
}
static int decode_refuse(const DecodeCall &d, const DecodePlan &p) {
    switch (p.refusal) {
        case DREF_PACKED_ONLY:
            set_error("decoder_forward: a LLMIE_DEC_PACKED_ONLY engine decodes on the packed kernels only (batch <= %d, no path switch)",
                      packed_rows_max(d.cfg));
            break;
        case DREF_LORA: set_error("decoder_forward: %s", kLoraRefusal); break;
// ... 110 lines not shown
        } else if (rope_ok && !fp8) {
            const int route = plan_linear_wq(linear_call(wqbits, T, H, QKV, EPI_NONE_, c.int4_group, x, qw, qsc, ws, nullptr, nullptr, nullptr,
                                                         nullptr, slabs, ws, lc.deq_bytes)).route;
            if (route == LR_W8_G8P && gemm256_qkv_rope_eligible(G256_W8, T, QKV, H, x, qw, qsc, ws)) o.qkv = PQ_ROPE_W8;
            if (route == LR_WQ_IMAGE_PREFILL && gemm256_qkv_rope_eligible(G256_F16, T, QKV, H, x, ws, nullptr, ws)) o.qkv = PQ_ROPE_IMAGE;
        }
        const bool gu_fused8 = fp8 && gemm256_swiglu_fills(T, 2 * I) && H % 128 == 0 && lc.mis_gu_w == 0;
        const LinearCall gc = linear_call(wqbits ? wqbits : 16, T, H, 2 * I, EPI_SWIGLU_, c.int4_group, x, gw, gsc, ws, nullptr, nullptr, nullptr, nullptr,
                                          slabs, wqbits ? ws : nullptr, lc.deq_bytes);
        if (nq && gu_fused8 && lc.ffn_gamma && lc.mis_gu_scale == 0) o.ffn_norm = PN_QUANT, o.gate_up = PG_E4M3_SWIGLU;
        else if (fp8) o.gate_up = gu_fused8 ? PG_FP8_SWIGLU : PG_TWO_LAUNCH;
        else if (wqbits) o.gate_up = (T < kWqPrefillRows || gemm256_swiglu_fills(T, 2 * I)) && plan_linear_wq(gc).route != LR_REFUSED ? PG_FUSED : PG_TWO_LAUNCH;
        else o.gate_up = plan_linear_f16(gc).route != LR_REFUSED ? PG_FUSED : PG_TWO_LAUNCH;
    }
    o.rope_done = o.qkv == PQ_ROPE_F16 || o.qkv == PQ_ROPE_W8 || o.qkv == PQ_ROPE_IMAGE || o.qkv == PQ_ROPE_E4M3 || o.qkv == PQ_ROPE_UNPACKED ||
                  o.qkv == PQ_SPLITK_ROPE;
    o.attn = plan_prefill_attn(batch, max_q_len, c.head_num, c.kv_fmt == LLMIE_KV_FP8, o.rope_done);
    for (int op : {LLMIE_OP_ATTN_NORM, LLMIE_OP_QKV_GEMM, LLMIE_OP_MHA, LLMIE_OP_O_GEMM, LLMIE_OP_FFN_NORM, LLMIE_OP_GATE_UP_SWIGLU, LLMIE_OP_DOWN_GEMM})
        o.launches[op] = 1;
    if (o.qkv == PQ_ROPE_UNPACKED || o.qkv == PQ_SPLITK || o.qkv == PQ_SPLITK_ROPE) o.launches[LLMIE_OP_QKV_GEMM] = 2;
    if (o.gate_up == PG_TWO_LAUNCH || o.gate_up == PG_UNPACK_TWO_LAUNCH || o.gate_up == PG_SPLITK) o.launches[LLMIE_OP_GATE_UP_SWIGLU] = 2;
    if (path == PP_LORA)
        for (int op : {LLMIE_OP_QKV_GEMM, LLMIE_OP_O_GEMM, LLMIE_OP_GATE_UP_SWIGLU, LLMIE_OP_DOWN_GEMM}) o.launches[op] += 2;
    return o;
}
static PrefillCall prefill_call_of_flags(const llmie_decoder_config &cfg, int tokens, unsigned call_flags, const EngineSwitches &sw) {
    return PrefillCall{cfg, tokens, !(call_flags & LLMIE_PLAN_WEIGHTS_MISALIGNED), !(call_flags & LLMIE_PLAN_SCALES_MISALIGNED),
                       !(call_flags & (LLMIE_PLAN_HIDDEN_MISALIGNED | LLMIE_PLAN_GAMMAS_MISALIGNED)), (call_flags & LLMIE_PLAN_O_BIAS) != 0, sw,
                       (call_flags & LLMIE_PLAN_LORA) != 0};
}

extern "C" const char *llmie_decoder_plan_name(const llmie_decoder_config *cfg, int prefill, int rows, unsigned call_flags,
                                               unsigned switch_mask) {
    if (!config_ok(cfg)) {
        set_error("decoder_plan_name: invalid config");
        return nullptr;
    }
    if ((cfg->flags & LLMIE_DEC_PACKED_ONLY) && !packed_wf(cfg)) {
        set_error("%s", packed_only_refusal(cfg));
        return nullptr;
    }
    const EngineSwitches sw = switches_of_mask(switch_mask);
    if (prefill) {
        if (rows < 1) {
            set_error("decoder_plan_name: %d tokens", rows);
            return nullptr;
        }
        const PrefillPlan p = plan_prefill(prefill_call_of_flags(*cfg, rows, call_flags, sw));
        if (p.path == PP_REFUSED) return (void)prefill_refuse(p), nullptr;
        return prefill_path_name(p.path);
    }
    if (rows < 1 || rows > cfg->max_batch) {
        set_error("decoder_forward: batch %d outside [1,%d]", rows, cfg->max_batch);
        return nullptr;
    }
    const DecodeCall dc{*cfg, rows, (call_flags & LLMIE_PLAN_PAGED) != 0, (call_flags & LLMIE_PLAN_RAGGED) != 0,
                        (call_flags & LLMIE_PLAN_HIDDEN_MISALIGNED) ? 8u : 0u, (call_flags & LLMIE_PLAN_WEIGHTS_MISALIGNED) ? 8u : 0u, sw,
                        (call_flags & LLMIE_PLAN_LORA) != 0};
    const DecodePlan p = plan_decode(dc);
    if (p.path == DP_REFUSED) return (void)decode_refuse(dc, p), nullptr;
    return decode_path_name(p.path);
}

static KvView kv_view(const llmie_decoder_config &c, void *k, void *v, const int32_t *block_table, int max_pages, int num_pages) {
    const bool fp8 = c.kv_fmt == LLMIE_KV_FP8;
    return KvView{k, v, block_table, max_pages, num_pages, fp8 ? 1 : 0, (fp8 && c.k_scale > 0.f) ? c.k_scale : 1.f,
                  (fp8 && c.v_scale > 0.f) ? c.v_scale : 1.f};
}

struct DecodeStep {
    llmie_decoder *dec;
    const llmie_decoder_config &c;
    void *h;
    int batch;
    KvView kv;
    DecodePos pos;
    llmie_stream stream;
    hipStream_t st;
    int H, QKV, I, wbits;
    bool fp8;
    llmie_dtype dt;

    int attention(const void *qkv, const void *qkv_bias, void *out, int layer, const SplitKSlabs *qkv_slabs = nullptr,
                  const SlabScale *qkv_scale = nullptr, int out_x32 = 0, bool rope = true) const {
        return decoder_mha_rope(DecodeAttnShape{batch, c.head_num, c.kv_head_num, c.head_size, c.max_seq_len, dt},
                                DecodeAttnIo{qkv, qkv_bias, out, dec->attn_ws, dec->attn_ws_bytes, rope ? dec->rope_table : nullptr,
                                             rope ? c.rotary_dim : 0, nullptr, qkv_slabs, qkv_scale, out_x32},
                                kv, pos, layer, st);
    }

    int gemv() const {
        int rc;
        auto lin = [&](const void *x, const llmie_matrix &w, void *y, int K, int N, int epi, const void *residual,
                       const void *gamma, const void *pre_bias) -> int {
            if (fp8) {
                if (ksplit_eligible(batch, K, 8))
                    return linear_fp8_gemv((const half_t *)x, (const uint8_t *)w.data, (const float *)w.scale, (half_t *)y, batch,
                                           K, N, epi, nullptr, (const half_t *)residual, (const half_t *)gamma,
                                           (const half_t *)pre_bias, c.rms_eps, st);
                return linear_fp8((const half_t *)x, (const uint8_t *)w.data, (const float *)w.scale, (half_t *)y, batch, K, N, nullptr,
                                  (const half_t *)residual, dec->fp8_ws, dec->fp8_ws_bytes, dec->slab_ws, st);
            }
            if (wbits == 16) {
                if (gamma)
                    return linear_f16_nk_norm((const half_t *)x, (const half_t *)w.data, (half_t *)y, batch, K, N, epi, nullptr,
                                              (const half_t *)residual, (const half_t *)gamma, (const half_t *)pre_bias,
                                              c.rms_eps, st);
                return linear_f16_nk((const half_t *)x, (const half_t *)w.data, (half_t *)y, batch, K, N, epi, nullptr,
                                     (const half_t *)residual, dec->slab_ws, st);
            }
            return linear_wq(wbits, (const half_t *)x, w.data, (const half_t *)w.scale, (half_t *)y, batch, K, N, c.int4_group,
                             epi, nullptr, (const half_t *)residual, (const half_t *)gamma, (const half_t *)pre_bias,
                             c.rms_eps, dec->slab_ws, st);
        };
        for (int l = 0; l < c.num_layers; ++l) {
            const llmie_layer_weights &w = dec->layers[l];
            TIMED(LLMIE_OP_QKV_GEMM, lin(h, w.qkv, dec->qkv, H, QKV, EPI_NONE_, nullptr, w.attn_norm_gamma, nullptr));
            TIMED(LLMIE_OP_MHA, attention(dec->qkv, w.qkv.bias, dec->mha, l));
            TIMED(LLMIE_OP_O_GEMM, lin(dec->mha, w.o, h, H, H, EPI_NONE_, h, nullptr, nullptr));
            TIMED(LLMIE_OP_GATE_UP_SWIGLU, lin(h, w.gate_up, dec->act, H, 2 * I, EPI_SWIGLU_, nullptr, w.ffn_norm_gamma, w.o.bias));
            TIMED(LLMIE_OP_DOWN_GEMM, lin(dec->act, w.down, h, I, H, EPI_NONE_, h, nullptr, nullptr));
        }
        return LLMIE_OK;
    }

    int packed() const {
        int rc;
        const int wf = dec->pk_wf;
        half_t *hh = static_cast<half_t *>(h);
        half_t *qkvb = reinterpret_cast<half_t *>(dec->qkv);
        for (int l = 0; l < c.num_layers; ++l) {
            const llmie_layer_weights &w = dec->layers[l];
            const llmie_decoder::PackedLayer &pw = dec->packed[l];
            const bool first = l == 0, last = l + 1 == c.num_layers;
            TIMED(LLMIE_OP_QKV_GEMM, pk_linear(wf, first ? hh : dec->hx, pw.qkv, pw.sc[0] ? pw.sc[0] : w.qkv.scale, qkvb, batch, H, QKV, PKE_PLAIN, first ? 0 : PKX_X,
                                               nullptr, static_cast<const half_t *>(w.attn_norm_gamma), nullptr, c.rms_eps, nullptr, 0, st));
            TIMED(LLMIE_OP_MHA, attention(dec->qkv, w.qkv.bias, dec->mhax, l, nullptr, nullptr, 1));
            TIMED(LLMIE_OP_O_GEMM, pk_linear(wf, dec->mhax, pw.o, pw.sc[1] ? pw.sc[1] : w.o.scale, dec->hx, batch, H, H, PKE_PLAIN, PKX_X | PKX_Y | (first ? 0 : PKX_RES),
                                             first ? hh : dec->hx, nullptr, nullptr, 0.f, nullptr, 0, st));
            TIMED(LLMIE_OP_GATE_UP_SWIGLU, pk_linear(wf, dec->hx, pw.gate_up, pw.sc[2] ? pw.sc[2] : w.gate_up.scale, dec->actx, batch, H, 2 * I, PKE_SWIGLU, PKX_X | PKX_Y,
                                                     nullptr, static_cast<const half_t *>(w.ffn_norm_gamma), static_cast<const half_t *>(w.o.bias),
                                                     c.rms_eps, nullptr, 0, st));
            TIMED(LLMIE_OP_DOWN_GEMM, pk_linear(wf, dec->actx, pw.down, pw.sc[3] ? pw.sc[3] : w.down.scale, last ? hh : dec->hx, batch, I, H, PKE_PLAIN,
                                                PKX_X | PKX_RES | (last ? 0 : PKX_Y), dec->hx, nullptr, nullptr, 0.f, dec->pk_slab,
                                                dec->pk_slab_floats, st));
        }
        return LLMIE_OK;
    }
    bool chain_joins() const {
        if (!dec->pk_sync) return false;
        const int wf = dec->pk_wf;
        half_t *qkvb = reinterpret_cast<half_t *>(dec->qkv);
        const llmie_layer_weights &w = dec->layers[0];
        const llmie_decoder::PackedLayer &pw = dec->packed[0];
        PkChain ch;
        pk_chain_begin(&ch, wf, batch);
        return ch.ok &&
                !pk_chain_add(&ch, 0, dec->mhax, pw.o, pw.sc[1] ? pw.sc[1] : w.o.scale, dec->hx, H, H, PKE_PLAIN, PKX_X | PKX_Y | PKX_RES, dec->hx, nullptr, nullptr, 0.f, nullptr, 0) &&
                !pk_chain_add(&ch, 1, dec->hx, pw.gate_up, pw.sc[2] ? pw.sc[2] : w.gate_up.scale, dec->actx, H, 2 * I, PKE_SWIGLU, PKX_X | PKX_Y, nullptr,
                              static_cast<const half_t *>(w.ffn_norm_gamma), static_cast<const half_t *>(w.o.bias), c.rms_eps, nullptr, 0) &&
                !pk_chain_add(&ch, 2, dec->actx, pw.down, pw.sc[3] ? pw.sc[3] : w.down.scale, dec->hx, I, H, PKE_PLAIN, PKX_X | PKX_RES | PKX_Y, dec->hx, nullptr, nullptr,
                              0.f, dec->pk_slab, dec->pk_slab_floats) &&
                (c.num_layers == 1 ||
                 !pk_chain_add(&ch, 4, dec->hx, pw.qkv, pw.sc[0] ? pw.sc[0] : w.qkv.scale, qkvb, H, QKV, PKE_PLAIN, PKX_X, nullptr,
                               static_cast<const half_t *>(w.attn_norm_gamma), nullptr, c.rms_eps, nullptr, 0));
    }
    int packed_chain() const {
        int rc;
        const int wf = dec->pk_wf;
        half_t *hh = static_cast<half_t *>(h);
        half_t *qkvb = reinterpret_cast<half_t *>(dec->qkv);
        for (int l = 0; l < c.num_layers; ++l) {
            const llmie_layer_weights &w = dec->layers[l];
            const llmie_decoder::PackedLayer &pw = dec->packed[l];
            const bool first = l == 0, last = l + 1 == c.num_layers;
            if (first)
                TIMED(LLMIE_OP_QKV_GEMM, pk_linear(wf, hh, pw.qkv, pw.sc[0] ? pw.sc[0] : w.qkv.scale, qkvb, batch, H, QKV, PKE_PLAIN, 0, nullptr,
                                                   static_cast<const half_t *>(w.attn_norm_gamma), nullptr, c.rms_eps, nullptr, 0, st));
            TIMED(LLMIE_OP_MHA, attention(dec->qkv, w.qkv.bias, dec->mhax, l, nullptr, nullptr, 1));
            PkChain ch;
            pk_chain_begin(&ch, wf, batch);
            rc = pk_chain_add(&ch, 0, dec->mhax, pw.o, pw.sc[1] ? pw.sc[1] : w.o.scale, dec->hx, H, H, PKE_PLAIN, PKX_X | PKX_Y | (first ? 0 : PKX_RES),
                              first ? hh : dec->hx, nullptr, nullptr, 0.f, nullptr, 0);
            if (!rc) rc = pk_chain_add(&ch, 1, dec->hx, pw.gate_up, pw.sc[2] ? pw.sc[2] : w.gate_up.scale, dec->actx, H, 2 * I, PKE_SWIGLU, PKX_X | PKX_Y, nullptr,
                                       static_cast<const half_t *>(w.ffn_norm_gamma), static_cast<const half_t *>(w.o.bias), c.rms_eps, nullptr, 0);
            if (!rc) rc = pk_chain_add(&ch, 2, dec->actx, pw.down, pw.sc[3] ? pw.sc[3] : w.down.scale, last ? hh : dec->hx, I, H, PKE_PLAIN,
                                       PKX_X | PKX_RES | (last ? 0 : PKX_Y), dec->hx, nullptr, nullptr, 0.f, dec->pk_slab, dec->pk_slab_floats);
            if (!rc && !last) {
                const llmie_layer_weights &wn = dec->layers[l + 1];
                const llmie_decoder::PackedLayer &pn = dec->packed[l + 1];
                rc = pk_chain_add(&ch, 4, dec->hx, pn.qkv, pn.sc[0] ? pn.sc[0] : wn.qkv.scale, qkvb, H, QKV, PKE_PLAIN, PKX_X, nullptr,
                                  static_cast<const half_t *>(wn.attn_norm_gamma), nullptr, c.rms_eps, nullptr, 0);
            }
            if (rc) return rc;
            ch.stamps = dec->pk_stamps;
            TIMED(LLMIE_OP_CHAIN, pk_chain_launch(&ch, dec->pk_sync + static_cast<size_t>(l) * (pk_chain_sync_bytes() / sizeof(unsigned)), dec->pk_err, st));
        }
        return LLMIE_OK;
    }

    int splitk() const {
        int rc;
// ... 748 lines not shown
```

### llm-inference-engine_amd/csrc/gemm_kernels.cuh

```cuda
#pragma once
#include "device_utils.cuh"

namespace llmie {

enum : int { EPI_NONE = 0, EPI_SWIGLU = 1 };


struct GemvArgs {
    const half_t *x;
    const void *W;
    half_t *y;
    int K, N;
    const half_t *bias;
    const half_t *residual;
    const half_t *gamma;
    const half_t *pre_bias;
    float eps;
    int epi, norm;
    const void *scale;
    int group;
};


template <int WBITS> struct WFmt;
template <> struct WFmt<16> { static constexpr int XE = 1; };
template <> struct WFmt<8> { static constexpr int XE = 2; };
template <> struct WFmt<4> { static constexpr int XE = 4; };

__device__ __forceinline__ half2_t as_half2(unsigned int u) { return __builtin_bit_cast(half2_t, u); }

template <int WBITS, bool FP8 = false>
__device__ __forceinline__ float chunk_dot(const uint4_t w, const half8_t (&x)[WFmt<WBITS>::XE], float acc) {
    if constexpr (WBITS == 16) {
        return dot8(__builtin_bit_cast(half8_t, w), x[0], acc);
    } else if constexpr (WBITS == 8 && FP8) {
#pragma unroll
        for (int i = 0; i < 4; ++i) {
            const half2_t wlo = __builtin_amdgcn_cvt_scalef32_pk_f16_fp8(static_cast<int>(w[i]), 1.0f, false);
            const half2_t whi = __builtin_amdgcn_cvt_scalef32_pk_f16_fp8(static_cast<int>(w[i]), 1.0f, true);
            const half8_t xv = x[i >> 1];
            const int b = (i & 1) * 4;
            acc = __builtin_amdgcn_fdot2(wlo, half2_t{xv[b], xv[b + 1]}, acc, false);
            acc = __builtin_amdgcn_fdot2(whi, half2_t{xv[b + 2], xv[b + 3]}, acc, false);
        }
        return acc;
    } else if constexpr (WBITS == 8) {
#pragma unroll
        for (int i = 0; i < 4; ++i) {
            const unsigned int v = w[i] ^ 0x80808080u;
            const unsigned int lo = __builtin_amdgcn_perm(0x64646464u, v, 0x04010400u);
            const unsigned int hi = __builtin_amdgcn_perm(0x64646464u, v, 0x04030402u);
            const half2_t wlo = as_half2(lo), whi = as_half2(hi);
            const half8_t xv = x[i >> 1];
            const int b = (i & 1) * 4;
            acc = __builtin_amdgcn_fdot2(wlo, half2_t{xv[b], xv[b + 1]}, acc, false);
            acc = __builtin_amdgcn_fdot2(whi, half2_t{xv[b + 2], xv[b + 3]}, acc, false);
        }
        return acc;
    } else {
#pragma unroll
        for (int i = 0; i < 4; ++i) {
            const half8_t xv = x[i];
            const unsigned int w0 = w[i], w8 = w[i] >> 8;
            const half2_t h0 = as_half2((w0 & 0x000F000Fu) | 0x64006400u);
            const half2_t h1 = as_half2((w0 & 0x00F000F0u) | 0x64006400u);
            const half2_t h2 = as_half2((w8 & 0x000F000Fu) | 0x64006400u);
            const half2_t h3 = as_half2((w8 & 0x00F000F0u) | 0x64006400u);
            acc = __builtin_amdgcn_fdot2(h0, half2_t{xv[0], xv[1]}, acc, false);
            acc = __builtin_amdgcn_fdot2(h1, half2_t{xv[2], xv[3]}, acc, false);
            acc = __builtin_amdgcn_fdot2(h2, half2_t{xv[4], xv[5]}, acc, false);
            acc = __builtin_amdgcn_fdot2(h3, half2_t{xv[6], xv[7]}, acc, false);
        }
        return acc;
    }
}
__device__ __forceinline__ half8_t prescale_x_int4(const half8_t v) {
    const float s = 0.0625f;
    return half8_t{v[0], v[1], from_f32<half_t>(to_f32(v[2]) * s), from_f32<half_t>(to_f32(v[3]) * s),
                   v[4], v[5], from_f32<half_t>(to_f32(v[6]) * s), from_f32<half_t>(to_f32(v[7]) * s)};
}
__device__ __forceinline__ float int4_offset_term(const half8_t v) {
    return 1032.0f * (to_f32(v[0]) + to_f32(v[1]) + to_f32(v[4]) + to_f32(v[5])) +
           1152.0f * (to_f32(v[2]) + to_f32(v[3]) + to_f32(v[6]) + to_f32(v[7]));
}
__device__ __forceinline__ half8_t permute_x_int4(const half8_t v) {
    return half8_t{v[0], v[4], v[1], v[5], v[2], v[6], v[3], v[7]};
}

template <int M, int RPW, int XC, int WBITS, bool DB = false, bool FP8 = false, int RI = 1>
__global__ __launch_bounds__(256) void gemv_ksplit_kernel(const GemvArgs a) {
    static_assert(RPW % 2 == 0, "rows come in pairs");
    constexpr int XE = WFmt<WBITS>::XE;
    constexpr int EPC = 8 * XE;
    __shared__ float red[2][4][M * RPW];
    __shared__ float ssq[4][M];
    const int K = a.K, N = a.N;
    const int nch = K / EPC;
    const int nx8 = K >> 3;
    const size_t row_bytes = static_cast<size_t>(K) * WBITS / 8;
    static_assert(RI == 1 || RI == 2, "one or two rows per workgroup instruction");
    const int tid = threadIdx.x, lane = tid & 63, wave = tid >> 6;
    constexpr int TPR = 256 / RI, WPR = 4 / RI;
    const int sub = tid / TPR, ct = tid % TPR;
    const bool swiglu = a.epi == EPI_SWIGLU;
    const int half_n = N >> 1;
    const int out_n = swiglu ? half_n : N;
    const int ngroups = swiglu ? (half_n + (RPW / 2) * RI - 1) / ((RPW / 2) * RI) : (N + RPW * RI - 1) / (RPW * RI);
    auto row_of = [&](int grp, int r) {
        int row = swiglu ? (grp * (RPW / 2) + (r >> 1)) * RI + sub + (r & 1) * half_n : (grp * RPW + r) * RI + sub;
        const int lim = swiglu ? ((r & 1) ? N : half_n) : N;
        return row < lim ? row : lim - 1;
    };

    half8_t xr[M][XC][XE];
    const half8_t *xg = reinterpret_cast<const half8_t *>(a.x);
#pragma unroll
    for (int m = 0; m < M; ++m)
#pragma unroll
        for (int j = 0; j < XC; ++j) {
            const int cc = j * TPR + ct;
#pragma unroll
            for (int e = 0; e < XE; ++e)
                xr[m][j][e] = cc < nch ? xg[m * nx8 + cc * XE + e] : half8_t{0, 0, 0, 0, 0, 0, 0, 0};
        }
    half8_t g[XC][XE];
    if (a.norm) {
        const half8_t *gm = reinterpret_cast<const half8_t *>(a.gamma);
#pragma unroll
        for (int j = 0; j < XC; ++j) {
            const int cc = j * TPR + ct;
#pragma unroll
            for (int e = 0; e < XE; ++e) g[j][e] = cc < nch ? gm[cc * XE + e] : half8_t{0, 0, 0, 0, 0, 0, 0, 0};
        }
    }
    constexpr int SR = WBITS == 4 ? RPW : 1, SX = WBITS == 4 ? XC : 1;
    uint4_t wbA[RPW][XC], wbB[DB ? RPW : 1][DB ? XC : 1];
    half_t wscA[SR][SX], wscB[DB ? SR : 1][DB ? SX : 1];
    const unsigned char *Wb = reinterpret_cast<const unsigned char *>(a.W);
    const half_t *scale = reinterpret_cast<const half_t *>(a.scale);
    const int sgroups = (WBITS == 4) ? K / a.group : 1;
    auto load_group = [&](int grp, auto &wb, auto &wsc) {
#pragma unroll
        for (int r = 0; r < RPW; ++r) {
            const uint4_t *w = reinterpret_cast<const uint4_t *>(Wb + static_cast<size_t>(row_of(grp, r)) * row_bytes);
            if constexpr (WBITS == 4) {
                const half_t *srow = scale + static_cast<size_t>(row_of(grp, r)) * sgroups;
#pragma unroll
                for (int j = 0; j < XC; ++j) wsc[r][j] = srow[(min(j * TPR + ct, nch - 1) * EPC) / a.group];
            }
#pragma unroll
            for (int j = 0; j < XC; ++j) {
                const int cc = min(j * TPR + ct, nch - 1);
                wb[r][j] = load_nt(w + cc);
            }
        }
    };
    int grp = blockIdx.x;
    if (grp < ngroups) load_group(grp, wbA, wscA);

    if (a.norm) {
        const half8_t *pb = reinterpret_cast<const half8_t *>(a.pre_bias);
        if (pb) {
#pragma unroll
            for (int j = 0; j < XC; ++j) {
                const int cc = j * TPR + ct;
                if (cc < nch) {
#pragma unroll
                    for (int e = 0; e < XE; ++e) {
                        const half8_t b = pb[cc * XE + e];
#pragma unroll
                        for (int m = 0; m < M; ++m)
#pragma unroll
                            for (int i = 0; i < 8; ++i) xr[m][j][e][i] = from_f32<half_t>(to_f32(xr[m][j][e][i]) + to_f32(b[i]));
                    }
                }
            }
        }
#pragma unroll
        for (int m = 0; m < M; ++m) {
            float ss = 0.f;
#pragma unroll
            for (int j = 0; j < XC; ++j)
#pragma unroll
                for (int e = 0; e < XE; ++e) ss = dot8(xr[m][j][e], xr[m][j][e], ss);
            ss = wave_sum(ss);
            if (lane == 0) ssq[wave][m] = ss;
        }
        __syncthreads();
#pragma unroll
        for (int m = 0; m < M; ++m) {
            const float inv = rsqrtf((RI == 1 ? ssq[0][m] + ssq[1][m] + ssq[2][m] + ssq[3][m] : ssq[0][m] + ssq[1][m]) / static_cast<float>(K) + a.eps);
#pragma unroll
            for (int j = 0; j < XC; ++j)
#pragma unroll
                for (int e = 0; e < XE; ++e)
#pragma unroll
                    for (int i = 0; i < 8; ++i)
                        xr[m][j][e][i] = from_f32<half_t>(to_f32(xr[m][j][e][i]) * to_f32(g[j][e][i]) * inv);
        }
    }
    if constexpr (WBITS == 4) {
#pragma unroll
        for (int m = 0; m < M; ++m)
#pragma unroll
            for (int j = 0; j < XC; ++j)
#pragma unroll
                for (int e = 0; e < XE; ++e) xr[m][j][e] = prescale_x_int4(permute_x_int4(xr[m][j][e]));
    }
    float xcorr4[WBITS == 4 ? M : 1][WBITS == 4 ? XC : 1];
    if constexpr (WBITS == 4) {
#pragma unroll
        for (int m = 0; m < M; ++m)
#pragma unroll
            for (int j = 0; j < XC; ++j) {
                float t = 0.f;
#pragma unroll
                for (int e = 0; e < XE; ++e) t += int4_offset_term(xr[m][j][e]);
                xcorr4[m][j] = -t;
            }
    }
    __shared__ float amx[FP8 ? 4 : 1][M], xscale_sh[M];
    if constexpr (FP8) {
#pragma unroll
        for (int m = 0; m < M; ++m) {
            float amax = 0.f;
#pragma unroll
            for (int j = 0; j < XC; ++j)
#pragma unroll
                for (int e = 0; e < XE; ++e)
#pragma unroll
                    for (int i = 0; i < 8; ++i) amax = fmaxf(amax, fabsf(to_f32(xr[m][j][e][i])));
            amax = wave_max(amax);
            if (lane == 0) amx[wave][m] = amax;
        }
        __syncthreads();
#pragma unroll
        for (int m = 0; m < M; ++m) {
            const float amax = fmaxf(fmaxf(amx[0][m], amx[1][m]), fmaxf(amx[2][m], amx[3][m]));
            const float sc = amax > 0.f ? amax / 448.0f : 1.0f;
            if (tid == 0) xscale_sh[m] = sc;
#pragma unroll
            for (int j = 0; j < XC; ++j)
#pragma unroll
// ... 20 lines not shown
            for (int j = 0; j < XC; ++j)
#pragma unroll
                for (int e = 0; e < XE; ++e)
#pragma unroll
                    for (int i = 0; i < 8; ++i) sx += to_f32(xr[m][j][e][i]);
            xcorr[m] = -1152.0f * sx;
        }
    }
    auto step = [&](auto &wb, auto &wsc, auto &wbn, auto &wscn, const int cur, const int it) {
        const int nxt = cur + gridDim.x;
        if constexpr (DB) {
            if (nxt < ngroups) load_group(nxt, wbn, wscn);
        }
        float acc[M][RPW];
#pragma unroll
        for (int r = 0; r < RPW; ++r) {
            float sc[XC];
            if constexpr (WBITS == 4) {
#pragma unroll
                for (int j = 0; j < XC; ++j) sc[j] = to_f32(wsc[r][j]);
            }
#pragma unroll
            for (int m = 0; m < M; ++m) {
                float sdot = xcorr[m];
#pragma unroll
                for (int j = 0; j < XC; ++j) {
                    if constexpr (WBITS == 4) sdot = fmaf(sc[j], chunk_dot<4>(wb[r][j], xr[m][j], xcorr4[m][j]), sdot);
                    else sdot = chunk_dot<WBITS, FP8>(wb[r][j], xr[m][j], sdot);
                }
                acc[m][r] = sdot;
            }
        }
        if constexpr (!DB) {
            if (nxt < ngroups) load_group(nxt, wb, wsc);
        }
#pragma unroll
        for (int r = 0; r < RPW; ++r)
#pragma unroll
            for (int m = 0; m < M; ++m) acc[m][r] = wave_sum(acc[m][r]);
        float *slot = &red[it & 1][0][0];
        if (lane == 0) {
#pragma unroll
            for (int m = 0; m < M; ++m)
#pragma unroll
                for (int r = 0; r < RPW; ++r) slot[wave * (M * RPW) + m * RPW + r] = acc[m][r];
        }
        __syncthreads();
        auto row_scale = [&](int row) {
            if constexpr (FP8) return reinterpret_cast<const float *>(a.scale)[row];
            else return (WBITS == 8) ? to_f32(scale[row]) : 1.0f;
        };
        if (swiglu) {
            if (tid < M * (RPW / 2) * RI) {
                const int m = tid / ((RPW / 2) * RI), qh = tid % ((RPW / 2) * RI), q = qh / RI, h = qh % RI;
                const int col = (cur * (RPW / 2) + q) * RI + h;
                if (col < half_n) {
                    float gt = 0.f, up = 0.f;
#pragma unroll
                    for (int w = 0; w < WPR; ++w) {
                        gt += slot[(h * WPR + w) * (M * RPW) + m * RPW + 2 * q];
                        up += slot[(h * WPR + w) * (M * RPW) + m * RPW + 2 * q + 1];
                    }
                    gt *= row_scale(col) * (FP8 ? xscale_sh[m] : 1.0f);
                    up *= row_scale(col + half_n) * (FP8 ? xscale_sh[m] : 1.0f);
                    a.y[static_cast<size_t>(m) * out_n + col] = from_f32<half_t>((gt / (1.0f + expf(-gt))) * up);
                }
            }
        } else {
            if (tid < M * RPW * RI) {
                const int m = tid / (RPW * RI), rh = tid % (RPW * RI), r = rh / RI, h = rh % RI;
                const int col = (cur * RPW + r) * RI + h;
                if (col < N) {
                    float v = 0.f;
#pragma unroll
                    for (int w = 0; w < WPR; ++w) v += slot[(h * WPR + w) * (M * RPW) + m * RPW + r];
                    v *= row_scale(col) * (FP8 ? xscale_sh[m] : 1.0f);
                    if (a.bias) v += to_f32(a.bias[col]);
                    if (a.residual) v += to_f32(a.residual[static_cast<size_t>(m) * N + col]);
                    a.y[static_cast<size_t>(m) * N + col] = from_f32<half_t>(v);
                }
            }
        }
    };
    for (int it = 0; grp < ngroups;) {
        step(wbA, wscA, wbB, wscB, grp, it);
        grp += gridDim.x;
        ++it;
        if constexpr (DB) {
            if (grp < ngroups) {
                step(wbB, wscB, wbA, wscA, grp, it);
                grp += gridDim.x;
                ++it;
            }
        }
    }
}

template <int M>
__global__ __launch_bounds__(256) void gemv_lds_kernel(const GemvArgs a) {
    constexpr int U = 8;
    extern __shared__ __attribute__((aligned(16))) unsigned char smem_raw[];
    half8_t *xs = reinterpret_cast<half8_t *>(smem_raw);
    __shared__ float inv_rms[M];
    const int K = a.K, N = a.N;
    const int nch = K >> 3, total = M * nch;
    const int tid = threadIdx.x, lane = tid & 63, wave = tid >> 6;
    const bool swiglu = a.epi == EPI_SWIGLU;
    {
        const half8_t *xg = reinterpret_cast<const half8_t *>(a.x);
        const half8_t *pb = reinterpret_cast<const half8_t *>(a.pre_bias);
        for (int i = tid; i < total; i += 256) {
            half8_t v = xg[i];
            if (a.norm && pb) {
                const half8_t b = pb[i % nch];
#pragma unroll
                for (int e = 0; e < 8; ++e) v[e] = from_f32<half_t>(to_f32(v[e]) + to_f32(b[e]));
            }
            xs[i] = v;
        }
    }
    __syncthreads();
    if (a.norm) {
        for (int m = wave; m < M; m += 4) {
            float ss = 0.f;
            for (int c = lane; c < nch; c += 64) {
                const half8_t v = xs[m * nch + c];
                ss = dot8(v, v, ss);
            }
            ss = wave_sum(ss);
            if (lane == 0) inv_rms[m] = rsqrtf(ss / static_cast<float>(K) + a.eps);
        }
        __syncthreads();
        const half8_t *gm = reinterpret_cast<const half8_t *>(a.gamma);
        for (int i = tid; i < total; i += 256) {
            const int m = i / nch, c = i - m * nch;
            half8_t v = xs[i];
            const half8_t g = gm[c];
            const float sc = inv_rms[m];
#pragma unroll
            for (int e = 0; e < 8; ++e) v[e] = from_f32<half_t>(to_f32(v[e]) * to_f32(g[e]) * sc);
            xs[i] = v;
        }
        __syncthreads();
    }
    const int half_n = N >> 1;
    const int npairs = swiglu ? half_n : ((N + 1) >> 1);
    for (int pair = blockIdx.x * 4 + wave; pair < npairs; pair += gridDim.x * 4) {
        const int r0 = swiglu ? pair : 2 * pair;
        const int r1 = swiglu ? pair + half_n : min(2 * pair + 1, N - 1);
        const half8_t *w0 = reinterpret_cast<const half8_t *>(static_cast<const half_t *>(a.W) + static_cast<size_t>(r0) * K);
        const half8_t *w1 = reinterpret_cast<const half8_t *>(static_cast<const half_t *>(a.W) + static_cast<size_t>(r1) * K);
        float acc0[M], acc1[M];
#pragma unroll
        for (int m = 0; m < M; ++m) acc0[m] = acc1[m] = 0.f;
        for (int c = lane; c < nch; c += 64 * U) {
            half8_t a0[U], a1[U];
#pragma unroll
            for (int u = 0; u < U; ++u) {
                const int cc = c + 64 * u;
                if (cc < nch) {
                    a0[u] = load_nt(w0 + cc);
                    a1[u] = load_nt(w1 + cc);
                }
            }
#pragma unroll
            for (int u = 0; u < U; ++u) {
                const int cc = c + 64 * u;
// ... 534 lines not shown
```

### llm-inference-engine_amd/csrc/linear.hip

```cpp
#include "gemm_kernels.cuh"
#include "gemm256.cuh"
#include "gemm8p.cuh"
#include "gemm_mid.cuh"
#include "llmie_internal.h"

#include <algorithm>
#include <cstdlib>

namespace llmie {

template <int M, int RPW, int XC, int WBITS, bool DB = false, bool FP8 = false, int RI = 1> static void launch_ksplit(const GemvArgs &a, hipStream_t st) {
    const bool swiglu = a.epi == EPI_SWIGLU;
    const int groups = swiglu ? (a.N / 2 + (RPW / 2) * RI - 1) / ((RPW / 2) * RI) : (a.N + RPW * RI - 1) / (RPW * RI);
    constexpr int target = (WBITS == 16 || WBITS == 4) ? 512 : 768;
    const int iters = (groups + target - 1) / target;
    const int grid = (groups + iters - 1) / iters;
    gemv_ksplit_kernel<M, RPW, XC, WBITS, DB, FP8, RI><<<grid, 256, 0, st>>>(a);
}

static int ksplit_xc(int K, int wbits) { return (K * wbits / 128 + 255) / 256; }

struct KsplitForm {
    int xc, rpw;
};
constexpr int kKsplitForms = 5;
constexpr KsplitForm ksplit_form_at(int wbits, bool fp8, int i) {
    constexpr KsplitForm f16[kKsplitForms] = {{1, 8}, {2, 4}, {4, 4}, {6, 4}, {8, 2}};
    constexpr KsplitForm q[kKsplitForms] = {{1, 8}, {2, 4}, {3, 2}, {0, 0}, {0, 0}};
    if (wbits == 16) return f16[i];
    if (i == 0 && wbits == 8 && !fp8) return KsplitForm{1, 4};
    return q[i];
}
static int ksplit_form(int M, int K, int wbits) {
    if (M < 1 || M > 8 || K % (128 / wbits) != 0) return -1;
    const int xe = wbits == 16 ? 1 : (wbits == 8 ? 2 : 4);
    const int xc = ksplit_xc(K, wbits);
    for (int i = 0; i < kKsplitForms; ++i) {
        const KsplitForm f = ksplit_form_at(wbits, false, i);
        if (f.xc && xc <= f.xc) return M * f.xc * xe <= 16 ? i : -1;
    }
    return -1;
}
bool ksplit_eligible(int M, int K, int wbits) { return ksplit_form(M, K, wbits) >= 0; }

template <int M, int WBITS, bool FP8, int I> static void launch_ksplit_form(const GemvArgs &a, hipStream_t st) {
    constexpr KsplitForm f = ksplit_form_at(WBITS, FP8, I);
    if constexpr (f.xc != 0 && M * f.xc * WFmt<WBITS>::XE <= 16) {
        if constexpr (WBITS == 4 && I == 0) {
            if (a.K * WBITS / 128 <= 128 && (a.epi != EPI_SWIGLU || (a.N / 2) % 2 == 0)) {
                launch_ksplit<M, 8, 1, WBITS, true, FP8, 2>(a, st);
                return;
            }
        }
        launch_ksplit<M, f.rpw, f.xc, WBITS, WBITS != 16, FP8>(a, st);
    }
}
template <int M, int WBITS, bool FP8 = false> static void dispatch_ksplit(int form, const GemvArgs &a, hipStream_t st) {
    switch (form) {
        case 0: launch_ksplit_form<M, WBITS, FP8, 0>(a, st); break;
        case 1: launch_ksplit_form<M, WBITS, FP8, 1>(a, st); break;
        case 2: launch_ksplit_form<M, WBITS, FP8, 2>(a, st); break;
        case 3: launch_ksplit_form<M, WBITS, FP8, 3>(a, st); break;
        case 4: launch_ksplit_form<M, WBITS, FP8, 4>(a, st); break;
        default: break;
    }
}

static int gemv_f16_route(int M, int K) {
    if (K % 8 || M < 1 || M > 8) return LR_REFUSED;
    if (ksplit_form(M, K, 16) >= 0) return LR_GEMV_KSPLIT;
    return static_cast<size_t>(M) * K * 2 <= 64 * 1024 ? LR_GEMV_LDS : LR_REFUSED;
}

template <int M> static void dispatch_gemv_m(const GemvArgs &a, hipStream_t st) {
    const int form = ksplit_form(M, a.K, 16);
    if (form >= 0) return dispatch_ksplit<M, 16>(form, a, st);
    const bool swiglu = a.epi == EPI_SWIGLU;
    const int npairs = swiglu ? a.N / 2 : (a.N + 1) / 2;
    int wgs = (npairs + 3) / 4;
    if (wgs > 2048) wgs = 2048;
    gemv_lds_kernel<M><<<wgs, 256, static_cast<size_t>(M) * a.K * sizeof(half_t), st>>>(a);
}

static void dispatch_gemv(int M, const GemvArgs &a, hipStream_t st) {
    switch (M) {
        case 1: return dispatch_gemv_m<1>(a, st);
        case 2: return dispatch_gemv_m<2>(a, st);
        case 3: return dispatch_gemv_m<3>(a, st);
        case 4: return dispatch_gemv_m<4>(a, st);
        case 5: return dispatch_gemv_m<5>(a, st);
        case 6: return dispatch_gemv_m<6>(a, st);
        case 7: return dispatch_gemv_m<7>(a, st);
        case 8: return dispatch_gemv_m<8>(a, st);
        default: return;
    }
}

template <int WBITS, bool FP8 = false> static bool dispatch_gemv_q(int M, const GemvArgs &a, hipStream_t st) {
    const int form = ksplit_form(M, a.K, WBITS);
    if (form < 0) return false;
    switch (M) {
        case 1: dispatch_ksplit<1, WBITS, FP8>(form, a, st); break;
        case 2: dispatch_ksplit<2, WBITS, FP8>(form, a, st); break;
        case 3: dispatch_ksplit<3, WBITS, FP8>(form, a, st); break;
        case 4: dispatch_ksplit<4, WBITS, FP8>(form, a, st); break;
        case 5: dispatch_ksplit<5, WBITS, FP8>(form, a, st); break;
        case 6: dispatch_ksplit<6, WBITS, FP8>(form, a, st); break;
        case 7: dispatch_ksplit<7, WBITS, FP8>(form, a, st); break;
        default: dispatch_ksplit<8, WBITS, FP8>(form, a, st); break;
    }
    return true;
}
void gemv_q_launch(int wbits, int M, const GemvArgs &a, hipStream_t st) {
    if (wbits == 8) dispatch_gemv_q<8>(M, a, st);
    else dispatch_gemv_q<4>(M, a, st);
}
bool gemv_fp8_launch(int M, const GemvArgs &a, hipStream_t st) { return dispatch_gemv_q<8, true>(M, a, st); }

template <int EPI>
static void dispatch_skinny(int M, const half_t *x, const half_t *W, half_t *y, int K, int N,
                            const half_t *bias, const half_t *residual, hipStream_t st) {
    constexpr int NW = 8;
    const int mt = (M + 15) / 16;
    if constexpr (EPI == EPI_SWIGLU) {
        const int wgs = (N / 2 + 15) / 16;
        switch (mt) {
            case 1: skinny_mfma_f16_kernel<1, 2, NW, EPI><<<wgs, NW * 64, 0, st>>>(x, W, y, M, K, N, bias, residual); break;
            case 2: skinny_mfma_f16_kernel<2, 2, NW, EPI><<<wgs, NW * 64, 0, st>>>(x, W, y, M, K, N, bias, residual); break;
            case 3: skinny_mfma_f16_kernel<3, 2, NW, EPI><<<wgs, NW * 64, 0, st>>>(x, W, y, M, K, N, bias, residual); break;
            case 4: skinny_mfma_f16_kernel<4, 2, NW, EPI><<<wgs, NW * 64, 0, st>>>(x, W, y, M, K, N, bias, residual); break;
            default: break;
        }
    } else {
        const int tiles = (N + 15) / 16;
        switch (mt) {
            case 1: skinny_mfma_f16_kernel<1, 1, NW, EPI><<<tiles, NW * 64, 0, st>>>(x, W, y, M, K, N, bias, residual); break;
            case 2: skinny_mfma_f16_kernel<2, 2, NW, EPI><<<(tiles + 1) / 2, NW * 64, 0, st>>>(x, W, y, M, K, N, bias, residual); break;
            case 3: skinny_mfma_f16_kernel<3, 2, NW, EPI><<<(tiles + 1) / 2, NW * 64, 0, st>>>(x, W, y, M, K, N, bias, residual); break;
            case 4: skinny_mfma_f16_kernel<4, 2, NW, EPI><<<(tiles + 1) / 2, NW * 64, 0, st>>>(x, W, y, M, K, N, bias, residual); break;
            default: break;
        }
    }
}

template <typename T>
static void launch_generic(const T *a, const T *b, T *c, int batch, int M, int N, int K, bool trans_b,
                           const T *bias, const T *residual, hipStream_t st) {
    dim3 grid((N + 63) / 64, (M + 63) / 64, batch);
// ... 939 lines not shown
```

### llm-inference-engine_amd/csrc/llmie_internal.h

```cpp
#pragma once
#include "device_utils.cuh"

namespace llmie {

enum : int { EPI_NONE_ = 0, EPI_SWIGLU_ = 1 };

struct SlabWs {
    float *p;
    size_t floats;
};
size_t linear_splitk_ws_floats(int wbits, int M, int K, int N);

enum LinearRoute : int {
    LR_REFUSED = 0,
    LR_GEMV_KSPLIT, LR_GEMV_LDS, LR_SPLITK, LR_SPLITK_PASSES, LR_SKINNY, LR_SWIGLU256, LR_TILES256, LR_TILES256_PART, LR_TILES128, LR_GENERIC,
    LR_W8_G8P, LR_W8_G8P_SWIGLU, LR_W8_SPLITK_PASSES, LR_WQ_IMAGE_PREFILL, LR_WQ_IMAGE_LAST, LR_WQ_GEMV, LR_W4_SPLITK, LR_W4_CHUNKS,
    LR_W8_SPLITK, LR_W8_SKINNY,
    LR_MX4_GEMV, LR_MX4_MFMA, LR_MX4_CHUNKS,
};
enum LinearRefusal : int { LREF_NONE = 0, LREF_F16_SWIGLU, LREF_SLABS, LREF_W4_SPLITK, LREF_WQ_NORM, LREF_WQ_SWIGLU, LREF_WQ_SHAPE, LREF_MX4_SHAPE, LREF_MX4_EPI };
struct LinearCall {
    int bits, M, K, N, epi, group;
    bool bias, residual, gamma, pre_bias;
    unsigned mis_x, mis_w, mis_y, mis_bias, mis_residual, mis_gamma, mis_pre_bias, mis_scale, mis_image;
    bool slabs;
    size_t slab_floats;
    bool image;
    size_t image_bytes;
};
struct LinearPlan {
    int route;
    int refusal;
    size_t slab_floats;
    size_t image_bytes;
    int pass_rows;
    int inner;
};
inline unsigned mis16(const void *p) { return static_cast<unsigned>(reinterpret_cast<uintptr_t>(p) % 16); }
LinearCall linear_call_sizing(int bits, int M, int K, int N, int epi, int group = 128);
LinearCall linear_call(int bits, int M, int K, int N, int epi, int group, const void *x, const void *w, const void *scale, const void *y,
                       const void *bias, const void *residual, const void *gamma, const void *pre_bias, SlabWs ws, const void *image,
                       size_t image_bytes);
LinearPlan plan_linear_f16(const LinearCall &c);
LinearPlan plan_linear_wq(const LinearCall &c);
const char *linear_route_name(int route);
int linear_refuse(const LinearCall &c, const LinearPlan &p);
size_t linear_f16_reserve_slab_floats(int M, int K, int N);
int linear_f16_nk(const half_t *x, const half_t *W, half_t *y, int M, int K, int N, int epi,
                  const half_t *bias, const half_t *residual, SlabWs ws, hipStream_t st);

bool gemv_f16_eligible(int M, int K, const void *x, const void *W);
int linear_f16_nk_norm(const half_t *x, const half_t *W, half_t *y, int M, int K, int N, int epi, const half_t *bias,
                       const half_t *residual, const half_t *gamma, const half_t *pre_bias, float eps, hipStream_t st);

struct SplitKSlabs {
    float *slab;
    int KS, M, N;
};
enum : int { WF_FP8 = 108 };
enum : int { WF_MXFP4 = 204 };
int linear_splitk_partial(int wbits, const void *x, const void *W, int M, int K, int N, hipStream_t st, SplitKSlabs *out,
                          SlabWs ws, const half_t *gscale = nullptr );
int splitk_finalize(const SplitKSlabs &sk, const SlabScale &sc, half_t *y, int epi, const half_t *bias, const half_t *residual,
                    hipStream_t st);
bool splitk_rownorm_eligible(int N);
int splitk_rownorm(const SplitKSlabs &sk, const SlabScale &wscale, const half_t *bias, half_t *resid, const half_t *gamma,
                   float eps, half_t *y, uint8_t *xq, float *xscale, hipStream_t st);
bool rmsnorm_quant_eligible(int hidden);
int rmsnorm_quant_f16(const half_t *x, half_t *resid, const half_t *bias, const half_t *gamma, float eps, int tokens, int hidden,
                      bool fused, uint8_t *xq, float *xscale, hipStream_t st);
bool rmsnorm_oop_eligible(int hidden);
int rmsnorm_oop_f16(const half_t *x, half_t *y, const half_t *gamma, float eps, int tokens, int hidden, hipStream_t st);
int quantize_rows_fp8(const half_t *x, uint8_t *xq, float *xscale, int M, int K, hipStream_t st);
int linear_splitk(int wbits, const half_t *x, const void *W, const half_t *scale, half_t *y, int M, int K, int N, int epi,
                  const half_t *bias, const half_t *residual, SlabWs ws, hipStream_t st);
enum G256Operands : int { G256_F16 = 0, G256_E4M3 = 1, G256_W8 = 2 };
enum G256Form : int { G256_PLAIN = 0, G256_SWIGLU = 1, G256_QKV_ROPE = 2 };
struct G256Range {
    bool eight_phase;
    int width, col0, tiles;
};
struct G256Plan {
    int ranges;
    G256Range range[2];
};
G256Plan plan_gemm256(G256Form form, G256Operands ops, int M, int N, int K);
bool gemm256_fills(int M, int N);
bool gemm256_swiglu_fills(int M, int two_inter);
int gemm256_narrow_rounds(int M, int N);
bool gemm8p_fits(int N, int K, int elem_bytes);
void gemm256_launch(G256Operands ops, const void *x, const void *W, half_t *y, int M, int N, int K, const half_t *bias,
                    const half_t *residual, const float *xscale, const float *wscale, hipStream_t st);
void gemm256_swiglu_launch(G256Operands ops, const void *x, const void *W, half_t *y, int M, int two_inter, int K, const float *xscale,
                           const float *wscale, hipStream_t st);
bool gemm256_qkv_rope_eligible(G256Operands ops, int M, int N, int K, const void *x, const void *W, const void *wscale, const void *qkv);
void gemm256_qkv_rope_launch(G256Operands ops, const void *x, const void *W, half_t *qkv, int M, int N, int K, const float *xscale,
                             const float *wscale, const half_t *bias, const QkvRopeArgs *rap, int layer, hipStream_t st);
int dequantize_weights_f16(int wbits, const void *wq, const half_t *scale, half_t *w16, int N, int K, int group, hipStream_t st);
constexpr int kWqPrefillRows = 192;
size_t linear_wq_dequant_bytes(int wbits, int M, int K, int N);
struct WqWorkspace {
    void *deq;
    size_t deq_bytes;
    SlabWs slabs;
};
WqWorkspace wq_workspace(int wbits, int M, int K, int N, void *workspace, size_t workspace_bytes);
constexpr int kMx4GemvRows = 8, kMx4MfmaRows = 64;
int dequantize_mxfp4_f16(const uint8_t *wq, const uint8_t *scale, half_t *w16, int N, int K, hipStream_t st);
int linear_mxfp4(const half_t *x, const uint8_t *wq, const uint8_t *scale, half_t *y, int M, int K, int N, const half_t *bias,
                 const half_t *residual, void *image, size_t image_bytes, hipStream_t st);
struct GemvArgs;
bool ksplit_eligible(int M, int K, int wbits);
void gemv_q_launch(int wbits, int M, const GemvArgs &a, hipStream_t st);
bool gemv_fp8_launch(int M, const GemvArgs &a, hipStream_t st);
int linear_fp8_gemv(const half_t *x, const uint8_t *wq, const float *wscale, half_t *y, int M, int K, int N, int epi,
                    const half_t *bias, const half_t *residual, const half_t *gamma, const half_t *pre_bias, float eps,
                    hipStream_t st);
int linear_fp8(const half_t *x, const uint8_t *w_fp8, const float *w_scale, half_t *y, int M, int K, int N, const half_t *bias,
               const half_t *residual, void *act_ws, size_t act_ws_bytes, SlabWs slabs, hipStream_t st);
int linear_wq(int wbits, const half_t *x, const void *wq, const half_t *scale, half_t *y, int M, int K, int N, int group,
              int epi, const half_t *bias, const half_t *residual, const half_t *gamma, const half_t *pre_bias, float eps,
              SlabWs ws, hipStream_t st, void *deq = nullptr, size_t deq_bytes = 0);

enum : int { PKF_F16 = 16, PKF_I8 = 8, PKF_I4 = 4, PKF_FP8 = 108 };
enum : int { PKE_PLAIN = 0, PKE_SWIGLU = 1 };
enum : int { PKX_X = 1, PKX_Y = 2, PKX_RES = 4 };
size_t pk_packed_bytes(int wf, int N, int K, int swiglu);
size_t pk_packed_scale_bytes(int wf, int N, int K, int swiglu);
int pk_pack(int wf, const void *src, const void *src_scale, void *dst, void *dst_scale, int N, int K, int swiglu, hipStream_t st);
int pk_unpack_f16(int wf, const void *packed, const half_t *scale, half_t *w16, int N, int K, int swiglu, hipStream_t st);
bool pk_eligible(int wf, int M, int K, int N, int epi);
size_t pk_slab_floats(int wf, int M, int K, int N);
int pk_linear(int wf, const half_t *x, const void *Wp, const void *scale, half_t *y, int M, int K, int N, int epi, int x32_flags,
              const half_t *residual, const half_t *gamma, const half_t *pre_bias, float eps, float *slab_ws, size_t slab_ws_floats,
              hipStream_t st);
int x32_convert(const half_t *src, half_t *dst, int M, int K, int to_x32, hipStream_t st);
struct PkChain {
    int wf, M, nph, lds;
    bool ok;
    unsigned long long *stamps;
    alignas(16) unsigned char args[1024];
};
void pk_chain_begin(PkChain *ch, int wf, int M);
int pk_chain_add(PkChain *ch, int slot , const half_t *x, const void *Wp, const void *scale, half_t *y, int K, int N, int epi, int x32_flags,
                 const half_t *residual, const half_t *gamma, const half_t *pre_bias, float eps, float *slab_ws, size_t slab_ws_floats);
int pk_chain_launch(PkChain *ch, unsigned *sync, unsigned *err, hipStream_t st);
size_t pk_chain_sync_bytes();

struct KvView {
    void *k, *v;
    const int32_t *block_table;
    int max_pages, num_pages;
    int fp8;
    float k_scale, v_scale;
};
inline KvView kv_dense(void *k, void *v) { return KvView{k, v, nullptr, 0, 0, 0, 1.f, 1.f}; }
struct DecodePos {
    int step;
    const int32_t *step_dev;
    int ragged;
};
enum DecodeAttnKind : int { DA_REFUSED = 0, DA_SPLIT, DA_GENERIC };
enum DecodeAttnRefusal : int {
    DAREF_NONE = 0, DAREF_RAGGED_LENGTHS, DAREF_X32, DAREF_PAGES, DAREF_SLAB_ALIGNMENT, DAREF_E4M3_FORM, DAREF_E4M3, DAREF_WORKSPACE,
    DAREF_PAGED_GEOMETRY, DAREF_SLABS_GEOMETRY, DAREF_ROPE_GEOMETRY, DAREF_RAGGED_GEOMETRY, DAREF_GENERIC_SPAN,
};
struct DecodeAttnCall {
    llmie_dtype dtype;
    bool kv_e4m3, scales_positive;
    int head_size, head_num, kv_head_num, batch, max_seq_len;
    int step;
    bool step_dev, ragged;
    bool bias, rope, tickets, slabs, paged, out_x32;
    int max_pages, num_pages;
    unsigned mis_qkv, mis_bias, mis_k, mis_v;
    unsigned mis_slab, mis_wf, mis_wh8, slab_stride_mod4;
    bool workspace;
    size_t workspace_bytes;
};
struct DecodeAttnPlan {
    int kind, refusal;
    int hs, rep;
    bool e4m3;
    int cpw, chunk, grid[3], max_splits_ws;
    bool merge;
    int merge_grid[2], merge_block;
    size_t lds_bytes;
    size_t workspace_bytes;
};
DecodeAttnPlan plan_decode_attn(const DecodeAttnCall &c);
int decode_attn_refuse(const DecodeAttnCall &c, const DecodeAttnPlan &p);
struct DecodeAttnShape {
    int batch, head_num, kv_head_num, head_size, max_seq_len;
    llmie_dtype dtype;
};
struct DecodeAttnIo {
    const void *qkv, *qkv_bias;
    void *out, *workspace;
    size_t workspace_bytes;
    const float2 *rope;
    int rot_dim;
    int32_t *tickets;
    const SplitKSlabs *qkv_slabs;
    const SlabScale *qkv_scale;
    int out_x32;
};
int decoder_mha_rope(const DecodeAttnShape &g, const DecodeAttnIo &io, const KvView &kv, const DecodePos &pos, int layer, hipStream_t st);

int topk_round1_only(const void *probs, int32_t *tmp_ids, void *tmp_vals, int rows, int vocab, int K, int bpr, llmie_dtype dtype, hipStream_t st);
int decode_tail(const int32_t *tmp_ids, const void *tmp_vals, int32_t *ids, void *vals, int K, int bpr, int32_t *seq_len, uint8_t *finished,
                int32_t *out_id, int rows, int step, int32_t *step_dev, int end_id, int vocab, const void *embed, void *next_hidden, int hidden,
                int advance, unsigned *ticket, llmie_dtype dtype, hipStream_t st);

struct PrefillAttnPlan {
    int q_rows, waves, row_tiles;
    bool kv_e4m3;
    int grid[3];
    bool rope_append;
};
PrefillAttnPlan plan_prefill_attn(int batch, int max_q_len, int head_num, bool kv_e4m3, bool rope_done);
int prefill_attention_f16(const PrefillAttnPlan &plan, const KvView &kv, half_t *qkv, const half_t *qkv_bias, half_t *out,
                          const int32_t *cum_seqlens, const int32_t *history_len, const float2 *rope, int layer, int num_tokens,
                          int kv_head_num, int max_seq_len, int rotary_dim, hipStream_t st);
bool splitk_finalize_qkv_rope_eligible(const SplitKSlabs &sk, int head_size, const void *qkv, const void *bias);
int splitk_finalize_qkv_rope(const SplitKSlabs &sk, const SlabScale &sc, half_t *qkv, const half_t *qkv_bias, const KvView &kv,
                             const int32_t *cum_seqlens, const int32_t *history_len, const float2 *rope, int layer, int batch, int head_num,
                             int kv_head_num, int max_seq_len, int rotary_dim, hipStream_t st);
int prefill_token_table(const int32_t *cum_seqlens, const int32_t *history_len, int batch, int num_tokens, int32_t *tok_b, int32_t *tok_tpos,
                        QkvRopeArgs args, QkvRopeArgs *args_dev, hipStream_t st);

int sample_logits_check(const void *logits, int batch, int vocab, const llmie_sampling_params *params, const int32_t *history,
                        int history_stride, const int32_t *history_len, const int32_t *seq_len, const uint8_t *finished,
                        const int32_t *out_id, const void *workspace, size_t workspace_bytes, llmie_dtype dtype,
                        const char *entry = "sample_logits", bool own_workspace = true);
int sample_logits_launch(const void *logits, int batch, int vocab, const llmie_sampling_params *params, int32_t *history,
                         int history_stride, int32_t *history_len, int history_append, int32_t *seq_len, uint8_t *finished,
                         int32_t *out_id, float *out_logprob, int step, const int32_t *step_dev, int end_id, void *workspace,
                         llmie_dtype dtype, const void *embed, void *next_hidden, int hidden, int advance, unsigned *ticket,
                         hipStream_t st, const llmie_sampling_ext *ext = nullptr);
int sample_ext_check(int batch, int vocab, const llmie_sampling_ext *ext, bool *active, const char *entry = "sample_logits_ext");
size_t sample_logits_ws_row(int vocab);

}
```

Baseline: 382.8 tokens/s.

## Fold split-KV attention merge into O-projection GEMV via device hand-off

For batch-1 fp16 decode, the separate attention combine kernel is dropped. The O-projection k-split GEMV now has its first head_num workgroups merge the split-KV partials for one head each and publish the merged row, then bump an arrival counter. Every workgroup prefetches its weights while it waits for the counter, then runs the dot product, so one launch per layer disappears and the weight loads overlap with the merge. The scheme relies on all workgroups being resident at once (it is gated on CU count), adds a spin-wait with a timeout error word, and adds a memset per forward pass.

```diff
diff --git a/include/llmie.h b/include/llmie.h
--- a/include/llmie.h
+++ b/include/llmie.h
@@ -265,6 +265,7 @@
 
 #define LLMIE_DEC_NO_PACKED_COPY 1
 #define LLMIE_DEC_PACKED_ONLY 2
+#define LLMIE_DEC_NO_MERGE_HANDOFF 4
 size_t llmie_decoder_resident_weight_bytes(const llmie_decoder_config *cfg);
 
 #define LLMIE_PLAN_PAGED 1u
@@ -426,6 +427,7 @@
                               int *launches_by_op );
 
 int llmie_decoder_status(llmie_decoder *dec, llmie_stream stream);
+long long llmie_decoder_merge_handoffs(const llmie_decoder *dec);
 int llmie_decoder_debug_stamps(llmie_decoder *dec, void *stamps_dev);
 
 int llmie_advance_step(int32_t *step_dev, llmie_stream stream);
diff --git a/llm-inference-engine_amd/__init__.py b/llm-inference-engine_amd/__init__.py
--- a/llm-inference-engine_amd/__init__.py
+++ b/llm-inference-engine_amd/__init__.py
@@ -8,7 +8,7 @@
 W_F16, W_INT8, W_INT4, W_FP8, W_F32 = 0, 1, 2, 3, 4
 W_MXFP4 = 5
 KV_NATIVE, KV_FP8 = 0, 1
-DEC_NO_PACKED_COPY, DEC_PACKED_ONLY = 1, 2
+DEC_NO_PACKED_COPY, DEC_PACKED_ONLY, DEC_NO_MERGE_HANDOFF = 1, 2, 4
 ABI_VERSION = 3
 
 _lib = None
@@ -118,6 +118,7 @@
     "llmie_decoder_profile_begin": [_vp, _i],
     "llmie_decoder_profile_end": [_vp, _vp, _vp, _vp],
     "llmie_decoder_status": [_vp, _vp],
+    "llmie_decoder_merge_handoffs": [_vp],
     "llmie_decoder_resident_weight_bytes": [_vp],
     "llmie_decoder_repack": [_vp, _vp, _vp],
     "llmie_decoder_plan_name": [_vp, _i, _i, C.c_uint, C.c_uint],
@@ -128,6 +129,7 @@
     "llmie_target_arch": [],
 }
 _RESTYPES = {
+    "llmie_decoder_merge_handoffs": C.c_longlong,
     "llmie_decoder_mha_workspace_bytes": _sz,
     "llmie_decoder_resident_weight_bytes": _sz,
     "llmie_linear_fp8_workspace_bytes": _sz,
@@ -786,6 +788,9 @@
     def status(self):
         _check(lib().llmie_decoder_status(self.handle, _st()), "decoder_status")
 
+    def merge_handoffs(self):
+        return int(lib().llmie_decoder_merge_handoffs(self.handle))
+
     def close(self):
         if self.handle:
             lib().llmie_decoder_destroy(self.handle)
diff --git a/llm-inference-engine_amd/csrc/attention_decode.hip b/llm-inference-engine_amd/csrc/attention_decode.hip
--- a/llm-inference-engine_amd/csrc/attention_decode.hip
+++ b/llm-inference-engine_amd/csrc/attention_decode.hip
@@ -1,4 +1,5 @@
 #include "llmie_internal.h"
+#include "attn_merge.cuh"
 
 #include <cstdlib>
 #include <type_traits>
@@ -79,51 +80,9 @@
     int step_stride;
     int out_x32;
 };
-__device__ __forceinline__ int seq_step(const int32_t *step_dev, int step_arg, int stride, int b, int max_seq_len) {
-    const int s = step_dev ? step_dev[static_cast<size_t>(b) * stride] : step_arg;
-    return (s >= 1 && s <= max_seq_len) ? s : 0;
-}
 __device__ __forceinline__ size_t attn_out_index(int x32, int b, int k, int width) {
     if (!x32) return static_cast<size_t>(b) * width + k;
     return (static_cast<size_t>(k >> 5) * 2 + (b >> 4)) * 512 + ((k & 31) >> 3) * 128 + (b & 15) * 8 + (k & 7);
-}
-
-__device__ __forceinline__ void merge_round(const float (&ms)[16], const float (&ls)[16], const float (&os)[16], int s0, int nsplits,
-                                            float &M, float &L, float &o) {
-    float Mc = M;
-#pragma unroll
-    for (int i = 0; i < 16; ++i)
-        if (s0 + i < nsplits) Mc = fmaxf(Mc, ms[i]);
-    const float rescale = (M == -INFINITY) ? 0.f : __expf(M - Mc);
-    L *= rescale;
-    o *= rescale;
-#pragma unroll
-    for (int i = 0; i < 16; ++i)
-        if (s0 + i < nsplits) {
-            const float f = __expf(ms[i] - Mc);
-            L = fmaf(f, ls[i], L);
-            o = fmaf(f, os[i], o);
-        }
-    M = Mc;
-}
-__device__ __forceinline__ void merge_load(const float *__restrict__ p, int s0, int last, size_t stride, int d, float (&ms)[16],
-                                           float (&ls)[16], float (&os)[16]) {
-#pragma unroll
-    for (int i = 0; i < 16; ++i) {
-        const int s = min(s0 + i, last);
-        ms[i] = p[s * stride];
-        ls[i] = p[s * stride + 1];
-        os[i] = p[s * stride + 2 + d];
-    }
-}
-__device__ __forceinline__ float merge_splits(const float *__restrict__ p, int nsplits, size_t stride, int d) {
-    float M = -INFINITY, L = 0.f, o = 0.f;
-    for (int s0 = 0; s0 < nsplits; s0 += 16) {
-        float ms[16], ls[16], os[16];
-        merge_load(p, s0, nsplits - 1, stride, d, ms, ls, os);
-        merge_round(ms, ls, os, s0, nsplits, M, L, o);
-    }
-    return o / (L + 1e-6f);
 }
 
 template <typename T, int HS, int REP, int kAttnWaves = 4, int kAttnG = 8, typename KT = T>
@@ -727,6 +686,7 @@
     QkvSlabs qs;
     KvScale ks;
     PagedKv pg;
+    MergeHandoff *defer;
 };
 
 template <typename T, int HS, int REP, typename KT> static void launch_split(const DecodeAttnPlan &p, const DecodeAttnArgs &a, hipStream_t st) {
@@ -734,7 +694,12 @@
         static_cast<const T *>(a.qkv), static_cast<const T *>(a.bias), static_cast<KT *>(a.kc), static_cast<KT *>(a.vc), a.part,
         static_cast<T *>(a.out), a.head_num, a.kv_head_num, a.max_seq_len, a.step, a.step_dev, p.max_splits_ws, a.rope, a.rot_dim, a.tickets,
         a.qs, a.ks.k, a.ks.v, a.pg, p.cpw);
-    if (p.merge)
+    if (a.defer) a.defer->part = nullptr;
+    if (p.merge && a.defer && std::is_same<T, half_t>::value && p.grid[2] == 1 && !a.pg.step_stride && !a.pg.out_x32) {
+        MergeHandoff &d = *a.defer;
+        d.part = a.part, d.head_num = a.head_num, d.head_size = HS, d.chunk = p.chunk, d.max_splits = p.max_splits_ws;
+        d.max_seq_len = a.max_seq_len, d.step = a.step, d.step_dev = a.step_dev;
+    } else if (p.merge)
         decode_attn_combine_kernel<T><<<dim3(p.merge_grid[0], p.merge_grid[1]), p.merge_block, 0, st>>>(
             a.part, static_cast<T *>(a.out), a.head_num, HS, p.chunk, a.step, a.step_dev, p.max_splits_ws, a.pg.step_stride, a.max_seq_len,
             a.pg.out_x32);
@@ -787,7 +752,7 @@
     return DecodeAttnArgs{io.qkv, io.qkv_bias, static_cast<char *>(kv.k) + layer_bytes, static_cast<char *>(kv.v) + layer_bytes, io.out,
                           static_cast<float *>(io.workspace), g.head_num, g.kv_head_num, g.head_size, g.max_seq_len, pos.step, pos.step_dev,
                           io.rope, io.rot_dim, io.tickets, qs, KvScale{kv.k_scale, kv.v_scale},
-                          PagedKv{kv.block_table, kv.max_pages, pos.ragged ? 1 : 0, io.out_x32 ? 1 : 0}};
+                          PagedKv{kv.block_table, kv.max_pages, pos.ragged ? 1 : 0, io.out_x32 ? 1 : 0}, io.defer_merge};
 }
 static DecodeAttnCall decode_attn_call(const DecodeAttnShape &g, const DecodeAttnIo &io, const KvView &kv, const DecodePos &pos,
                                        const DecodeAttnArgs &a) {
diff --git a/llm-inference-engine_amd/csrc/attn_merge.cuh b/llm-inference-engine_amd/csrc/attn_merge.cuh
--- /dev/null
+++ b/llm-inference-engine_amd/csrc/attn_merge.cuh
@@ -0,0 +1,58 @@
+#pragma once
+#include "device_utils.cuh"
+
+namespace llmie {
+
+struct MergeHandoff {
+    const float *part;
+    int head_num, head_size, chunk, max_splits, max_seq_len;
+    int step;
+    const int32_t *step_dev;
+    unsigned *arrive;
+    unsigned *err;
+};
+
+__device__ __forceinline__ int seq_step(const int32_t *step_dev, int step_arg, int stride, int b, int max_seq_len) {
+    const int s = step_dev ? step_dev[static_cast<size_t>(b) * stride] : step_arg;
+    return (s >= 1 && s <= max_seq_len) ? s : 0;
+}
+
+__device__ __forceinline__ void merge_round(const float (&ms)[16], const float (&ls)[16], const float (&os)[16], int s0, int nsplits,
+                                            float &M, float &L, float &o) {
+    float Mc = M;
+#pragma unroll
+    for (int i = 0; i < 16; ++i)
+        if (s0 + i < nsplits) Mc = fmaxf(Mc, ms[i]);
+    const float rescale = (M == -INFINITY) ? 0.f : __expf(M - Mc);
+    L *= rescale;
+    o *= rescale;
+#pragma unroll
+    for (int i = 0; i < 16; ++i)
+        if (s0 + i < nsplits) {
+            const float f = __expf(ms[i] - Mc);
+            L = fmaf(f, ls[i], L);
+            o = fmaf(f, os[i], o);
+        }
+    M = Mc;
+}
+__device__ __forceinline__ void merge_load(const float *__restrict__ p, int s0, int last, size_t stride, int d, float (&ms)[16],
+                                           float (&ls)[16], float (&os)[16]) {
+#pragma unroll
+    for (int i = 0; i < 16; ++i) {
+        const int s = min(s0 + i, last);
+        ms[i] = p[s * stride];
+        ls[i] = p[s * stride + 1];
+        os[i] = p[s * stride + 2 + d];
+    }
+}
+__device__ __forceinline__ float merge_splits(const float *__restrict__ p, int nsplits, size_t stride, int d) {
+    float M = -INFINITY, L = 0.f, o = 0.f;
+    for (int s0 = 0; s0 < nsplits; s0 += 16) {
+        float ms[16], ls[16], os[16];
+        merge_load(p, s0, nsplits - 1, stride, d, ms, ls, os);
+        merge_round(ms, ls, os, s0, nsplits, M, L, o);
+    }
+    return o / (L + 1e-6f);
+}
+
+}
diff --git a/llm-inference-engine_amd/csrc/engine.hip b/llm-inference-engine_amd/csrc/engine.hip
--- a/llm-inference-engine_amd/csrc/engine.hip
+++ b/llm-inference-engine_amd/csrc/engine.hip
@@ -20,6 +20,12 @@
     size_t fp8_ws_bytes;
     SlabWs slab_ws;
     unsigned *tail_ticket = nullptr;
+    unsigned *ho_arrive = nullptr, *ho_err = nullptr;
+    size_t ho_arrive_bytes = 0;
+    long long ho_launches = 0;
+    ~llmie_decoder() {
+        if (ho_arrive) (void)hipFree(ho_arrive);
+    }
     struct PackedLayer {
         const unsigned char *qkv, *o, *gate_up, *down;
         const void *sc[4];
@@ -84,7 +90,7 @@
     if (c->dtype == LLMIE_F16 && c->wfmt == LLMIE_W_F32) return false;
     if (c->wfmt == LLMIE_W_MXFP4 && ((c->head_num * c->head_size) % 32 || c->inter_size % 32)) return false;
     if (c->kv_fmt != LLMIE_KV_NATIVE && c->kv_fmt != LLMIE_KV_FP8) return false;
-    if (c->flags & ~(LLMIE_DEC_NO_PACKED_COPY | LLMIE_DEC_PACKED_ONLY)) return false;
+    if (c->flags & ~(LLMIE_DEC_NO_PACKED_COPY | LLMIE_DEC_PACKED_ONLY | LLMIE_DEC_NO_MERGE_HANDOFF)) return false;
     if ((c->flags & LLMIE_DEC_NO_PACKED_COPY) && (c->flags & LLMIE_DEC_PACKED_ONLY)) return false;
     if (c->kv_fmt == LLMIE_KV_FP8) {
         const int rep = c->head_num / c->kv_head_num;
@@ -337,6 +343,14 @@
         delete d;
         return nullptr;
     }
+    d->ho_err = d->tail_ticket + 32;
+    d->ho_arrive_bytes = (static_cast<size_t>(cfg->num_layers) * sizeof(unsigned) + 15) & ~static_cast<size_t>(15);
+    if (hipMalloc(reinterpret_cast<void **>(&d->ho_arrive), d->ho_arrive_bytes) != hipSuccess ||
+        hipMemset(d->ho_arrive, 0, d->ho_arrive_bytes) != hipSuccess) {
+        set_error("decoder_create: allocating the hand-off words failed");
+        delete d;
+        return nullptr;
+    }
     d->fp8_ws = base + offs.fp8_ws;
     {
         const int kmax = cfg->inter_size > d->H ? cfg->inter_size : d->H;
@@ -450,6 +464,17 @@
         set_error("decoder_status: stream synchronise failed: %s", hipGetErrorString(hipGetLastError()));
         return LLMIE_ERR_LAUNCH;
     }
+    unsigned ho_word = 0;
+    if (hipMemcpy(&ho_word, dec->ho_err, sizeof(ho_word), hipMemcpyDeviceToHost) != hipSuccess) {
+        set_error("decoder_status: reading the device error word failed");
+        return LLMIE_ERR_LAUNCH;
+    }
+    if (ho_word) {
+        (void)hipMemset(dec->ho_err, 0, sizeof(ho_word));
+        set_error("decoder: the O projection's wait for the merged attention row timed out (code 0x%08x): a producer workgroup never "
+                  "arrived; the steps since are wrong; create the engine with LLMIE_DEC_NO_MERGE_HANDOFF to use the merge launch", ho_word);
+        return LLMIE_ERR_LAUNCH;
+    }
     if (!dec->pk_err) return LLMIE_OK;
     unsigned word = 0;
     if (hipMemcpy(&word, dec->pk_err, sizeof(word), hipMemcpyDeviceToHost) != hipSuccess) {
@@ -460,11 +485,13 @@
         (void)hipMemset(dec->pk_err, 0, sizeof(word));
         (void)hipMemset(dec->pk_sync, 0, static_cast<size_t>(dec->cfg.num_layers) * pk_chain_sync_bytes());
         set_error("decoder: a grid barrier of the persistent chain launch timed out (code 0x%08x, phase %u): not every workgroup was "
-                  "resident; set LLMIE_NO_CHAIN=1 to use the launch sequence", word, word & 0xfu);
+                  "resident; unset LLMIE_CHAIN to use the launch sequence", word, word & 0xfu);
         return LLMIE_ERR_LAUNCH;
     }
     return LLMIE_OK;
 }
+
+extern "C" long long llmie_decoder_merge_handoffs(const llmie_decoder *dec) { return dec ? dec->ho_launches : 0; }
 
 extern "C" int llmie_decoder_debug_stamps(llmie_decoder *dec, void *stamps_dev) {
     LLMIE_REQUIRE(dec, "decoder_debug_stamps: NULL decoder");
@@ -525,9 +552,10 @@
 struct EngineSwitches {
     bool no_fused_decode, no_fused_batch, no_packed_batch, chain, no_fused_short_prefill, no_qkv_rope_fusion;
 };
+static bool env_opt_in(const char *v) { return v && v[0] && !(v[0] == '0' && !v[1]); }
 static const EngineSwitches &engine_switches() {
     static const EngineSwitches s{getenv("LLMIE_NO_FUSED_DECODE") != nullptr,        getenv("LLMIE_NO_FUSED_BATCH") != nullptr,
-                                  getenv("LLMIE_NO_PACKED_BATCH") != nullptr,        getenv("LLMIE_CHAIN") != nullptr,
+                                  getenv("LLMIE_NO_PACKED_BATCH") != nullptr,        env_opt_in(getenv("LLMIE_CHAIN")),
                                   getenv("LLMIE_NO_FUSED_SHORT_PREFILL") != nullptr, getenv("LLMIE_NO_QKV_ROPE_FUSION") != nullptr};
     return s;
 }
@@ -804,10 +832,10 @@
     llmie_dtype dt;
 
     int attention(const void *qkv, const void *qkv_bias, void *out, int layer, const SplitKSlabs *qkv_slabs = nullptr,
-                  const SlabScale *qkv_scale = nullptr, int out_x32 = 0, bool rope = true) const {
+                  const SlabScale *qkv_scale = nullptr, int out_x32 = 0, bool rope = true, MergeHandoff *defer_merge = nullptr) const {
         return decoder_mha_rope(DecodeAttnShape{batch, c.head_num, c.kv_head_num, c.head_size, c.max_seq_len, dt},
                                 DecodeAttnIo{qkv, qkv_bias, out, dec->attn_ws, dec->attn_ws_bytes, rope ? dec->rope_table : nullptr,
-                                             rope ? c.rotary_dim : 0, nullptr, qkv_slabs, qkv_scale, out_x32},
+                                             rope ? c.rotary_dim : 0, nullptr, qkv_slabs, qkv_scale, out_x32, defer_merge},
                                 kv, pos, layer, st);
     }
 
@@ -835,11 +863,30 @@
                              epi, nullptr, (const half_t *)residual, (const half_t *)gamma, (const half_t *)pre_bias,
                              c.rms_eps, dec->slab_ws, st);
         };
+        const bool handoff = batch == 1 && wbits == 16 && !fp8 && !pos.ragged && !(c.flags & LLMIE_DEC_NO_MERGE_HANDOFF);
+        bool zeroed = false;
         for (int l = 0; l < c.num_layers; ++l) {
             const llmie_layer_weights &w = dec->layers[l];
+            MergeHandoff mh{};
+            const bool ho = handoff && linear_f16_handoff_eligible((const half_t *)dec->mha, (const half_t *)w.o.data, (const half_t *)h, H, H,
+                                                                   (const half_t *)h, c.head_num, c.head_size, dec->slab_ws);
+            if (ho && !zeroed) {
+                if (hipMemsetAsync(dec->ho_arrive, 0, dec->ho_arrive_bytes, st) != hipSuccess) {
+                    set_error("decoder_forward: clearing the hand-off words failed");
+                    return LLMIE_ERR_LAUNCH;
+                }
+                zeroed = true;
+            }
             TIMED(LLMIE_OP_QKV_GEMM, lin(h, w.qkv, dec->qkv, H, QKV, EPI_NONE_, nullptr, w.attn_norm_gamma, nullptr));
-            TIMED(LLMIE_OP_MHA, attention(dec->qkv, w.qkv.bias, dec->mha, l));
-            TIMED(LLMIE_OP_O_GEMM, lin(dec->mha, w.o, h, H, H, EPI_NONE_, h, nullptr, nullptr));
+            TIMED(LLMIE_OP_MHA, attention(dec->qkv, w.qkv.bias, dec->mha, l, nullptr, nullptr, 0, true, ho ? &mh : nullptr));
+            if (mh.part) {
+                mh.arrive = dec->ho_arrive + l, mh.err = dec->ho_err;
+                TIMED(LLMIE_OP_O_GEMM, linear_f16_nk_handoff(mh, (const half_t *)dec->mha, (const half_t *)w.o.data, (half_t *)h, H, H,
+                                                             (const half_t *)h, st));
+                ++dec->ho_launches;
+            } else {
+                TIMED(LLMIE_OP_O_GEMM, lin(dec->mha, w.o, h, H, H, EPI_NONE_, h, nullptr, nullptr));
+            }
             TIMED(LLMIE_OP_GATE_UP_SWIGLU, lin(h, w.gate_up, dec->act, H, 2 * I, EPI_SWIGLU_, nullptr, w.ffn_norm_gamma, w.o.bias));
             TIMED(LLMIE_OP_DOWN_GEMM, lin(dec->act, w.down, h, I, H, EPI_NONE_, h, nullptr, nullptr));
         }
diff --git a/llm-inference-engine_amd/csrc/gemm_kernels.cuh b/llm-inference-engine_amd/csrc/gemm_kernels.cuh
--- a/llm-inference-engine_amd/csrc/gemm_kernels.cuh
+++ b/llm-inference-engine_amd/csrc/gemm_kernels.cuh
@@ -1,4 +1,5 @@
 #pragma once
+#include "attn_merge.cuh"
 #include "device_utils.cuh"
 
 namespace llmie {
@@ -21,6 +22,15 @@
     int group;
 };
 
+struct GemvHandoffArgs : GemvArgs {
+    MergeHandoff ho;
+};
+template <bool HO> struct GemvKernelArgs { using type = GemvArgs; };
+template <> struct GemvKernelArgs<true> { using type = GemvHandoffArgs; };
+constexpr unsigned kHandoffTimeoutCode = 0x4D0FF000u;
+typedef __attribute__((address_space(1))) unsigned short ho_gu16;
+typedef __attribute__((address_space(1))) unsigned ho_gu32;
+
 
 template <int WBITS> struct WFmt;
 template <> struct WFmt<16> { static constexpr int XE = 1; };
@@ -87,8 +97,9 @@
     return half8_t{v[0], v[4], v[1], v[5], v[2], v[6], v[3], v[7]};
 }
 
-template <int M, int RPW, int XC, int WBITS, bool DB = false, bool FP8 = false, int RI = 1>
-__global__ __launch_bounds__(256) void gemv_ksplit_kernel(const GemvArgs a) {
+template <int M, int RPW, int XC, int WBITS, bool DB = false, bool FP8 = false, int RI = 1, bool HO = false>
+__global__ __launch_bounds__(256) void gemv_ksplit_kernel(const typename GemvKernelArgs<HO>::type a) {
+    static_assert(!HO || (WBITS == 16 && !DB && !FP8 && RI == 1), "the hand-off form streams fp16 rows");
     static_assert(RPW % 2 == 0, "rows come in pairs");
     constexpr int XE = WFmt<WBITS>::XE;
     constexpr int EPC = 8 * XE;
@@ -114,17 +125,19 @@
 
     half8_t xr[M][XC][XE];
     const half8_t *xg = reinterpret_cast<const half8_t *>(a.x);
-#pragma unroll
-    for (int m = 0; m < M; ++m)
-#pragma unroll
-        for (int j = 0; j < XC; ++j) {
-            const int cc = j * TPR + ct;
-#pragma unroll
-            for (int e = 0; e < XE; ++e)
-                xr[m][j][e] = cc < nch ? xg[m * nx8 + cc * XE + e] : half8_t{0, 0, 0, 0, 0, 0, 0, 0};
-        }
+    if constexpr (!HO) {
+#pragma unroll
+        for (int m = 0; m < M; ++m)
+#pragma unroll
+            for (int j = 0; j < XC; ++j) {
+                const int cc = j * TPR + ct;
+#pragma unroll
+                for (int e = 0; e < XE; ++e)
+                    xr[m][j][e] = cc < nch ? xg[m * nx8 + cc * XE + e] : half8_t{0, 0, 0, 0, 0, 0, 0, 0};
+            }
+    }
     half8_t g[XC][XE];
-    if (a.norm) {
+    if (!HO && a.norm) {
         const half8_t *gm = reinterpret_cast<const half8_t *>(a.gamma);
 #pragma unroll
         for (int j = 0; j < XC; ++j) {
@@ -156,9 +169,79 @@
         }
     };
     int grp = blockIdx.x;
-    if (grp < ngroups) load_group(grp, wbA, wscA);
-
-    if (a.norm) {
+    constexpr int PG = HO ? (32 / (RPW * XC) > 0 ? 32 / (RPW * XC) : 1) : 1;
+    uint4_t wbP[PG][HO ? RPW : 1][HO ? XC : 1];
+    float hoB = 0.f, hoR = 0.f;
+    if constexpr (!HO) {
+        if (grp < ngroups) load_group(grp, wbA, wscA);
+    } else {
+        const MergeHandoff &ho = a.ho;
+        if (static_cast<int>(blockIdx.x) < ho.head_num) {
+            const int h = blockIdx.x, d = tid;
+            const size_t stride = static_cast<size_t>(ho.head_size) + 2;
+            const float *p = ho.part + static_cast<size_t>(h) * ho.max_splits * stride;
+            float ms[16], ls[16], os[16];
+            merge_load(p, 0, ho.max_splits - 1, stride, min(d, ho.head_size - 1), ms, ls, os);
+            const int pos = seq_step(ho.step_dev, ho.step, 0, 0, ho.max_seq_len);
+            const int nsplits = (pos + ho.chunk - 1) / ho.chunk;
+            if (nsplits > 1 && d < ho.head_size) {
+                float Mx = -INFINITY, L = 0.f, o = 0.f;
+                merge_round(ms, ls, os, 0, nsplits, Mx, L, o);
+                for (int s0 = 16; s0 < nsplits; s0 += 16) {
+                    merge_load(p, s0, nsplits - 1, stride, d, ms, ls, os);
+                    merge_round(ms, ls, os, s0, nsplits, Mx, L, o);
+                }
+                const half_t v = from_f32<half_t>(o / (L + 1e-6f));
+                __hip_atomic_store((ho_gu16 *)a.x + h * ho.head_size + d,
+                                   __builtin_bit_cast(unsigned short, v), __ATOMIC_RELAXED, __HIP_MEMORY_SCOPE_AGENT);
+            }
+            asm volatile("s_waitcnt vmcnt(0)" ::: "memory");
+            __syncthreads();
+            if (tid == 0) __hip_atomic_fetch_add((ho_gu32 *)ho.arrive, 1u, __ATOMIC_RELAXED, __HIP_MEMORY_SCOPE_AGENT);
+        }
+#pragma unroll
+        for (int pgi = 0; pgi < PG; ++pgi) {
+            if (grp + pgi * static_cast<int>(gridDim.x) < ngroups) {
+                load_group(grp + pgi * static_cast<int>(gridDim.x), wbP[pgi], wscA);
+            } else {
+#pragma unroll
+                for (int r = 0; r < RPW; ++r)
+#pragma unroll
+                    for (int j = 0; j < XC; ++j) wbP[pgi][r][j] = uint4_t{0u, 0u, 0u, 0u};
+            }
+        }
+        if (tid < PG * RPW) {
+            const int col = (static_cast<int>(blockIdx.x) + (tid / RPW) * static_cast<int>(gridDim.x)) * RPW + tid % RPW;
+            if (col < N) {
+                if (a.bias) hoB = to_f32(a.bias[col]);
+                if (a.residual) hoR = to_f32(a.residual[col]);
+            }
+        }
+        if (tid == 0) {
+            const unsigned long long t0 = __builtin_amdgcn_s_memrealtime();
+            while (__hip_atomic_load((ho_gu32 *)ho.arrive, __ATOMIC_RELAXED, __HIP_MEMORY_SCOPE_AGENT) !=
+                   static_cast<unsigned>(ho.head_num)) {
+                __builtin_amdgcn_s_sleep(2);
+                if (__builtin_amdgcn_s_memrealtime() - t0 > 100000000ull) {
+                    __hip_atomic_store((ho_gu32 *)ho.err, kHandoffTimeoutCode + 1u, __ATOMIC_RELAXED, __HIP_MEMORY_SCOPE_AGENT);
+                    break;
+                }
+            }
+        }
+        __syncthreads();
+        const __amdgpu_buffer_rsrc_t xrs = __builtin_amdgcn_make_buffer_rsrc(const_cast<half_t *>(a.x), 0, M * K * 2, 0x00020000);
+#pragma unroll
+        for (int m = 0; m < M; ++m)
+#pragma unroll
+            for (int j = 0; j < XC; ++j) {
+                const int cc = j * TPR + ct;
+                xr[m][j][0] = __builtin_bit_cast(half8_t, __builtin_amdgcn_raw_buffer_load_b128(xrs, cc < nch ? (m * nx8 + cc) * 16 : M * K * 2, 0, 16 ));
+            }
+        grp += PG * static_cast<int>(gridDim.x);
+        if (grp < ngroups) load_group(grp, wbA, wscA);
+    }
+
+    if (!HO && a.norm) {
         const half8_t *pb = reinterpret_cast<const half8_t *>(a.pre_bias);
         if (pb) {
 #pragma unroll
@@ -345,7 +428,40 @@
             }
         }
     };
-    for (int it = 0; grp < ngroups;) {
+    int it = 0;
+    if constexpr (HO) {
+        static_assert(!HO || M == 1, "the hand-off form is the batch-1 form");
+        __shared__ float redP[4][PG * RPW];
+        float accP[PG][RPW];
+#pragma unroll
+        for (int pgi = 0; pgi < PG; ++pgi)
+#pragma unroll
+            for (int r = 0; r < RPW; ++r) {
+                float sdot = xcorr[0];
+#pragma unroll
+                for (int j = 0; j < XC; ++j) sdot = chunk_dot<WBITS, FP8>(wbP[pgi][r][j], xr[0][j], sdot);
+                accP[pgi][r] = wave_sum(sdot);
+            }
+        if (lane == 0) {
+#pragma unroll
+            for (int pgi = 0; pgi < PG; ++pgi)
+#pragma unroll
+                for (int r = 0; r < RPW; ++r) redP[wave][pgi * RPW + r] = accP[pgi][r];
+        }
+        __syncthreads();
+        if (tid < PG * RPW) {
+            const int cur = static_cast<int>(blockIdx.x) + (tid / RPW) * static_cast<int>(gridDim.x), col = cur * RPW + tid % RPW;
+            if (cur < ngroups && col < N) {
+                float v = 0.f;
+#pragma unroll
+                for (int w = 0; w < 4; ++w) v += redP[w][tid];
+                if (a.bias) v += hoB;
+                if (a.residual) v += hoR;
+                a.y[col] = from_f32<half_t>(v);
+            }
+        }
+    }
+    for (; grp < ngroups;) {
         step(wbA, wscA, wbB, wscB, grp, it);
         grp += gridDim.x;
         ++it;
diff --git a/llm-inference-engine_amd/csrc/linear.hip b/llm-inference-engine_amd/csrc/linear.hip
--- a/llm-inference-engine_amd/csrc/linear.hip
+++ b/llm-inference-engine_amd/csrc/linear.hip
@@ -64,6 +64,46 @@
         case 4: launch_ksplit_form<M, WBITS, FP8, 4>(a, st); break;
         default: break;
     }
+}
+
+constexpr int kHandoffGrid = 256;
+static bool handoff_device_ok() {
+    static const bool ok = [] {
+        int dev = 0, cus = 0;
+        if (hipGetDevice(&dev) != hipSuccess || hipDeviceGetAttribute(&cus, hipDeviceAttributeMultiprocessorCount, dev) != hipSuccess) return false;
+        return cus >= kHandoffGrid;
+    }();
+    return ok;
+}
+static int handoff_grid(int N, int rpw) {
+    const int groups = (N + rpw - 1) / rpw, iters = (groups + kHandoffGrid - 1) / kHandoffGrid;
+    return (groups + iters - 1) / iters;
+}
+template <int I> static void launch_ksplit_handoff(const GemvHandoffArgs &a, hipStream_t st) {
+    constexpr KsplitForm f = ksplit_form_at(16, false, I);
+    gemv_ksplit_kernel<1, f.rpw, f.xc, 16, false, false, 1, true><<<handoff_grid(a.N, f.rpw), 256, 0, st>>>(a);
+}
+bool linear_f16_handoff_eligible(const half_t *x, const half_t *W, const half_t *y, int K, int N, const half_t *residual, int head_num,
+                                 int head_size, SlabWs ws) {
+    const LinearCall c = linear_call(16, 1, K, N, EPI_NONE, 0, x, W, nullptr, y, nullptr, residual, nullptr, nullptr, ws, nullptr, 0);
+    if (plan_linear_f16(c).route != LR_GEMV_KSPLIT) return false;
+    const int form = ksplit_form(1, K, 16);
+    if (form < 0 || form > 2) return false;
+    if (head_num < 1 || K != head_num * head_size || head_size % 64 || head_size > 256 || reinterpret_cast<uintptr_t>(x) % 128) return false;
+    return handoff_grid(N, ksplit_form_at(16, false, form).rpw) >= head_num && handoff_device_ok();
+}
+int linear_f16_nk_handoff(const MergeHandoff &ho, const half_t *x, const half_t *W, half_t *y, int K, int N, const half_t *residual,
+                          hipStream_t st) {
+    GemvHandoffArgs a;
+    static_cast<GemvArgs &>(a) = GemvArgs{x, W, y, K, N, nullptr, residual, nullptr, nullptr, 0.f, EPI_NONE, 0, nullptr, 0};
+    a.ho = ho;
+    switch (ksplit_form(1, K, 16)) {
+        case 0: launch_ksplit_handoff<0>(a, st); break;
+        case 1: launch_ksplit_handoff<1>(a, st); break;
+        case 2: launch_ksplit_handoff<2>(a, st); break;
+        default: set_error("linear(merge hand-off): K=%d has no hand-off form", K); return LLMIE_ERR_UNSUPPORTED;
+    }
+    return launch_status("linear(merge hand-off)");
 }
 
 static int gemv_f16_route(int M, int K) {
diff --git a/llm-inference-engine_amd/csrc/llmie_internal.h b/llm-inference-engine_amd/csrc/llmie_internal.h
--- a/llm-inference-engine_amd/csrc/llmie_internal.h
+++ b/llm-inference-engine_amd/csrc/llmie_internal.h
@@ -1,4 +1,5 @@
 #pragma once
+#include "attn_merge.cuh"
 #include "device_utils.cuh"
 
 namespace llmie {
@@ -48,6 +49,11 @@
 size_t linear_f16_reserve_slab_floats(int M, int K, int N);
 int linear_f16_nk(const half_t *x, const half_t *W, half_t *y, int M, int K, int N, int epi,
                   const half_t *bias, const half_t *residual, SlabWs ws, hipStream_t st);
+
+bool linear_f16_handoff_eligible(const half_t *x, const half_t *W, const half_t *y, int K, int N, const half_t *residual, int head_num,
+                                 int head_size, SlabWs ws);
+int linear_f16_nk_handoff(const MergeHandoff &ho, const half_t *x, const half_t *W, half_t *y, int K, int N, const half_t *residual,
+                          hipStream_t st);
 
 bool gemv_f16_eligible(int M, int K, const void *x, const void *W);
 int linear_f16_nk_norm(const half_t *x, const half_t *W, half_t *y, int M, int K, int N, int epi, const half_t *bias,
@@ -204,6 +210,7 @@
     const SplitKSlabs *qkv_slabs;
     const SlabScale *qkv_scale;
     int out_x32;
+    MergeHandoff *defer_merge = nullptr;
 };
 int decoder_mha_rope(const DecodeAttnShape &g, const DecodeAttnIo &io, const KvView &kv, const DecodePos &pos, int layer, hipStream_t st);
 
```

Result: no change. 386.5 tokens/s (median of 6 runs) (+1.0%).
